# gillette7/Abmarl

Measured on NVIDIA B200. Metric: agent-steps/sec (obs+reward+done) over batched envs, higher is better.
Workload: dtype i8/f64

## Files before the change

### abmarl_b200/csrc/bgw.cu

```cuda
#include <cuda_runtime.h>

#include <algorithm>
#include <cmath>
#include <cstdarg>
#include <cstdio>
#include <cstdlib>
#include <cstring>
#include <vector>

#define BGW_SMALL_KERNELS
#include "bgw_dev.cuh"
#include "bgw_fast.cuh"
#include "bgw_maze.cuh"
#include "bgw_jit.h"

namespace {

thread_local char g_err[2048] = "";

int fail(int code, const char *fmt, ...)
{
    va_list ap;
    va_start(ap, fmt);
    vsnprintf(g_err, sizeof(g_err), fmt, ap);
    va_end(ap);
    return code;
}

#define CUDA_OK(call)                                                                                  \
    do {                                                                                               \
        cudaError_t err__ = (call);                                                                    \
        if (err__ != cudaSuccess) return fail(2, "%s failed: %s", #call, cudaGetErrorString(err__));   \
    } while (0)

struct DeviceGuard {
    int prev = -1;
    explicit DeviceGuard(int dev) { if (cudaGetDevice(&prev) == cudaSuccess && prev != dev) cudaSetDevice(dev); else prev = -1; }
    ~DeviceGuard() { if (prev >= 0) cudaSetDevice(prev); }
};

int align16(int x) { return (x + 15) & ~15; }
int pow2ceil(int x) { int p = 1; while (p < x) p <<= 1; return p; }

}

static const void *observe_fast_fn(int R)
{
    switch (R) {
    case 1: return (const void *)bgw_observe_fast_kernel<1>;
    case 2: return (const void *)bgw_observe_fast_kernel<2>;
    case 3: return (const void *)bgw_observe_fast_kernel<3>;
    case 4: return (const void *)bgw_observe_fast_kernel<4>;
    case 5: return (const void *)bgw_observe_fast_kernel<5>;
    }
    return nullptr;
}

struct BgwEngine {
    int device = 0;
    GeneralStepFn step_fn = nullptr;
    bgwjit::Kernel jit;
    bgwjit::Kernel fast_jit;
    bool fast_jit_on = false;
    const void *fast_fn = nullptr;
    MazeParams maze{};
    bool maze_ok = false, maze_small = false;
    DevSpec ds{}, dsf{};
    FastSpec fs{};
    int threads_fast = 0;
    bool pdl = true;
    bool poisoned = false;
    bool chain_ok = false;
    bool rollout_fused = true;
    bool randomize_action_input = false;
    int16_t *order_buf = nullptr;
    bool use_device_layouts = true;
    uint32_t seq = 0;
    uint32_t *ticket_ring = nullptr;
    std::vector<uint32_t> ticket_next;
    int fast_shape = 0;
    const void *observe_fn = nullptr;
    int observe_grid = 0, observe_smem = 0;
    BgwDims dims{};
    BgwState st{};
    bool bound = false;
    int threads = 0;
    uint64_t launches = 0;
    std::vector<void *> allocs;
};

namespace {

template <typename T>
int upload(BgwEngine *h, const T *src, size_t n, const T **dst)
{
    void *p = nullptr;
    CUDA_OK(cudaMalloc(&p, std::max<size_t>(n, 1) * sizeof(T)));
    h->allocs.push_back(p);
    if (n) CUDA_OK(cudaMemcpy(p, src, n * sizeof(T), cudaMemcpyHostToDevice));
    *dst = (const T *)p;
    return 0;
}

void los_apply_host(uint8_t *mask, int R, int rd, int cd)
{
    const int n = 2 * R + 1;
    if (rd == 0 && cd == 0) return;
    if (cd != 0) {
        double du, dl;
        if (rd == 0) { du = dl = (cd > 0) ? (double)cd - 0.5 : (double)cd + 0.5; }
        else if ((rd > 0) == (cd > 0)) { du = (double)cd - 0.5; dl = (double)cd + 0.5; }
        else { du = (double)cd + 0.5; dl = (double)cd - 0.5; }
        volatile double ku = ((double)rd + 0.5) / du, kl = ((double)rd - 0.5) / dl;
        const int c0 = cd > 0 ? cd : -R, c1 = cd > 0 ? R : cd;
        const int r0 = rd > 0 ? rd : -R, r1 = rd < 0 ? rd : R;
        for (int c = c0; c <= c1; ++c) {
            volatile double up = ku * (double)c, lo = kl * (double)c;
            for (int r = r0; r <= r1; ++r) {
                if (c == cd && r == rd) continue;
                if (lo < (double)r && (double)r < up) mask[(r + R) * n + (c + R)] = 0;
            }
        }
    } else {
        const double d = rd > 0 ? (double)rd - 0.5 : (double)rd + 0.5;
        volatile double kl = ((double)cd - 0.5) / d, kr = ((double)cd + 0.5) / d;
        const int r0 = rd > 0 ? rd : -R, r1 = rd > 0 ? R : rd;
        for (int r = r0; r <= r1; ++r) {
            volatile double le = kl * (double)r, ri = kr * (double)r;
            for (int c = -R; c <= R; ++c) {
                if (c == cd && r == rd) continue;
                if (le < (double)c && (double)c < ri) mask[(r + R) * n + (c + R)] = 0;
            }
        }
    }
}

template <typename Scratch>
__global__ void bgw_layout_kernel(const MazeParams p, const BgwState st, int E, int env_offset, const uint8_t *env_mask, int only_done)
{
    __shared__ Scratch w;
    if (threadIdx.x != 0) return;
    for (int e = blockIdx.x; e < E; e += gridDim.x) {
        if (only_done ? !(st.env_flags[e] & BGW_ENV_ALL_DONE) : (env_mask && !env_mask[e])) continue;
        const int err = maze_layout(p, (uint32_t)(env_offset + e), st.episode[e] + 1u, w, st.layout + (size_t)e * p.A);
        if (err) st.error[e] = (uint32_t)err;
    }
}

int first_role(const BgwSpec *sp, int role)
{
    for (int a = 0; a < sp->n_agents; ++a) if (sp->role[a] == role) return a;
    return -1;
}

}

extern "C" {

const char *bgw_last_error(void) { return g_err; }
int bgw_abi_version(void) { return BGW_ABI_VERSION; }

int bgw_create(const BgwSpec *sp, int device, bgw_handle *out)
{
    if (!sp || !out) return fail(1, "bgw_create: null argument");
    *out = nullptr;
    if (sp->abi_version != BGW_ABI_VERSION) return fail(1, "bgw_create: ABI version %d, library has %d", sp->abi_version, BGW_ABI_VERSION);
    int ndev = 0;
    if (cudaGetDeviceCount(&ndev) != cudaSuccess || ndev == 0)
        return fail(2, "bgw_create: no CUDA device (this engine has no CPU fallback)");
    if (device < 0 || device >= ndev) return fail(1, "bgw_create: device %d out of range (%d devices)", device, ndev);
    const int A = sp->n_agents, H = sp->rows, W = sp->cols, HW = H * W;
    if (A < 1 || A > BGW_MAX_AGENTS) return fail(1, "bgw_create: n_agents %d not in 1..%d", A, BGW_MAX_AGENTS);
    if (H < 1 || W < 1 || HW > BGW_MAX_CELLS) return fail(1, "bgw_create: grid %dx%d not supported (at most %d cells)", H, W, BGW_MAX_CELLS);
    if (sp->n_envs < 1) return fail(1, "bgw_create: n_envs must be positive");

    BgwEngine *h = new BgwEngine();
    h->device = device;
    DeviceGuard guard(device);
    DevSpec &d = h->ds;
    auto bail = [&](int rc) { bgw_destroy(h); return rc; };

    d.H = H; d.W = W; d.HW = HW; d.A = A; d.E = sp->n_envs; d.env_offset = sp->env_offset;
    d.program = sp->program; d.move_actor = sp->move_actor; d.attack_actor = sp->attack_actor;
    d.observer = sp->observer; d.observe_self = sp->observe_self; d.done_mask = sp->done_mask;
    d.manager = sp->manager; d.ravel = sp->ravel_actions; d.no_overlap = sp->no_overlap_at_reset;
    d.stacked = sp->stacked_attacks; d.horizon = sp->horizon; d.auto_reset = sp->auto_reset;
    d.randomize_placement_order = sp->randomize_placement_order;
    d.seed = sp->seed;
    memcpy(d.reward, sp->reward, sizeof(d.reward));

    std::vector<int16_t> learner_of(A, -1), agent_of;
    std::vector<uint16_t> blk, blk_static, var, init_cell(A, BGW_NONE);
    int max_enc = 0, rmax_obs = 0, rmax_att = 0, n_ammo = 0, att_payload = 1;
    for (int a = 0; a < A; ++a) if (sp->encoding[a] > max_enc) max_enc = std::min((int)sp->encoding[a], BGW_MAX_ENCODING);
    if (sp->attack_actor < BGW_ATTACK_NONE || sp->attack_actor > BGW_ATTACK_SELECTIVE) return bail(fail(1, "bgw_create: unknown attack actor %d", sp->attack_actor));
    for (int a = 0; a < A; ++a) {
        const int e = sp->encoding[a];
        if (e < 1 || e > BGW_MAX_ENCODING) return bail(fail(1, "bgw_create: entity %d has encoding %d, must be 1..%d", a, e, BGW_MAX_ENCODING));
        if (sp->target && (sp->target[a] < -1 || sp->target[a] >= A)) return bail(fail(1, "bgw_create: entity %d names target %d, must be -1 or an entity index below %d", a, (int)sp->target[a], A));
        if (sp->klass[a] & BGW_AG_LEARNER) { learner_of[a] = (int16_t)agent_of.size(); agent_of.push_back((int16_t)a); }
        if (sp->klass[a] & BGW_AG_BLOCKING) {
            const bool is_static = !(sp->klass[a] & (BGW_AG_MOVING | BGW_AG_HEALTH)) && sp->init_row[a] >= 0;
            (is_static ? blk_static : blk).push_back((uint16_t)a);
        }
        if (sp->init_row[a] < 0) var.push_back((uint16_t)a);
        else {
            if (sp->init_row[a] >= H || sp->init_col[a] < 0 || sp->init_col[a] >= W)
                return bail(fail(1, "bgw_create: entity %d initial position off the grid", a));
            init_cell[a] = (uint16_t)(sp->init_row[a] * W + sp->init_col[a]);
        }
        if ((sp->klass[a] & BGW_AG_LEARNER) && (sp->klass[a] & BGW_AG_OBSERVING)) {
            int R = sp->view_range[a];
            if (R < 0) return bail(fail(1, "bgw_create: negative view range"));
            rmax_obs = std::max(rmax_obs, R);
        }
        if (sp->klass[a] & BGW_AG_AMMO) {
            ++n_ammo;
            if (!sp->initial_ammo || sp->initial_ammo[a] < 0) return bail(fail(1, "bgw_create: entity %d is an AmmoAgent without a non-negative initial_ammo", a));
        }
        if ((sp->klass[a] & BGW_AG_ATTACKING) && sp->attack_actor != BGW_ATTACK_NONE) {
            const int R = sp->attack_range[a], n = 2 * R + 1, sim = sp->simultaneous_attacks[a];
            rmax_att = std::max(rmax_att, R);
            if (R < 0) return bail(fail(1, "bgw_create: negative attack range"));
            if ((sp->program == BGW_PROG_TEAM_BATTLE || sp->program == BGW_PROG_REACH_TARGET) && sp->attack_actor == BGW_ATTACK_BINARY && sim > 1)
                return bail(fail(1, "bgw_create: TeamBattleSim.step with the BinaryAttackActor is only defined for simultaneous_attacks == 1 (team_battle_example.py:41)"));
            if (sim > BGW_MAX_SIMATT) return bail(fail(1, "bgw_create: simultaneous_attacks %d exceeds %d", sim, BGW_MAX_SIMATT));
            int w = 1, groups = 1;
            if (sp->attack_actor == BGW_ATTACK_ENCODING) { w = max_enc; groups = 0; for (int e = 1; e <= max_enc; ++e) groups += (int)((sp->attack_map[sp->encoding[a]] >> e) & 1); }
            else if (sp->attack_actor == BGW_ATTACK_RESTRICTED) { w = sim; groups = 1; }
            else if (sp->attack_actor == BGW_ATTACK_SELECTIVE) { w = n * n; groups = n * n; }
            if (n * n > 256 && sp->attack_actor >= BGW_ATTACK_RESTRICTED) return bail(fail(1, "bgw_create: attack range %d: a ravelled window cell must fit one byte (range <= 7)", R));
            if (groups * std::max(sim, 1) > BGW_MAX_VICTIMS)
                return bail(fail(1, "bgw_create: entity %d could attack %d agents in one step, the limit is %d", a, groups * sim, BGW_MAX_VICTIMS));
            att_payload = std::max(att_payload, w);
        }
    }
    const int L = (int)agent_of.size();
    if (L < 1) return bail(fail(1, "bgw_create: the simulation has no learning agent"));
    d.n_dyn_blk = (int)blk.size();
    blk.insert(blk.end(), blk_static.begin(), blk_static.end());
    d.L = L; d.max_enc = max_enc; d.n_blk = (int)blk.size(); d.n_var = (int)var.size();
    if (sp->attack_actor != BGW_ATTACK_NONE && d.n_blk > 0 && (2 * rmax_att + 1) * (2 * rmax_att + 1) > 32 * BGW_ATT_MASK_WORDS)
        return bail(fail(1, "bgw_create: attack_range %d with view-blocking entities exceeds the attacker's LOS mask (range <= 7)", rmax_att));
    if (sp->observer == BGW_OBS_STACKED && A > 127) return bail(fail(1, "bgw_create: stacked observer counts are int8 (at most 127 entities)"));
    if (sp->ravel_actions && sp->move_actor != BGW_MOVE_BOX) return bail(fail(1, "bgw_create: ravel_actions needs MoveActor"));

    d.a_nav = first_role(sp, BGW_ROLE_NAVIGATOR); d.a_target = first_role(sp, BGW_ROLE_TARGET);
    d.a_pacman = first_role(sp, BGW_ROLE_PACMAN); d.has_food = first_role(sp, BGW_ROLE_FOOD) >= 0;
    if (sp->program == BGW_PROG_MAZE && (d.a_nav < 0 || d.a_target < 0 || learner_of[d.a_nav] < 0))
        return bail(fail(1, "bgw_create: MazeNavigationSim needs a learning navigator and a target"));
    if (sp->program == BGW_PROG_MULTI_MAZE && d.a_target < 0) return bail(fail(1, "bgw_create: MultiMazeNavigationSim needs a target"));
    for (int k = 0; k < 10; ++k) d.a_script[k] = first_role(sp, BGW_ROLE_SCRIPTED_BADDIE + k);
    if ((sp->program == BGW_PROG_PACMAN || sp->program == BGW_PROG_PACMAN_SIMPLE) && (d.a_pacman < 0 || learner_of[d.a_pacman] < 0 || H <= 9 || W <= 20))
        return bail(fail(1, "bgw_create: PacmanSim needs a learning pacman and the (9,0)<->(9,20) tunnel (pacman.py:87-92)"));
    if (sp->program == BGW_PROG_REACH_TARGET && (d.a_target < 0 || learner_of[d.a_target] < 0))
        return bail(fail(1, "bgw_create: ReachTheTargetSim needs a learning target agent"));
    if (sp->program < BGW_PROG_TEAM_BATTLE || sp->program > BGW_PROG_USER) return bail(fail(1, "bgw_create: unknown program %d", sp->program));
    if (sp->program == BGW_PROG_USER && sp->manager == BGW_MANAGER_DYNAMIC_ORDER)
        return bail(fail(1, "bgw_create: a user step program cannot run under BGW_MANAGER_DYNAMIC_ORDER (its next_agent rule is built in)"));

    BgwDims &dm = h->dims;
    dm.n_envs = d.E; dm.n_agents = A; dm.n_learners = L;
    dm.obs_c = 1;
    if (sp->observer == BGW_OBS_ABSOLUTE) { dm.obs_h = H; dm.obs_w = W; }
    else dm.obs_h = dm.obs_w = 2 * rmax_obs + 1;
    if (sp->observer == BGW_OBS_STACKED) dm.obs_c = max_enc;
    const long long ncell = (long long)dm.obs_h * dm.obs_w * dm.obs_c;
    if (ncell > (1 << 24)) return bail(fail(1, "bgw_create: observation of %lld cells is too large", ncell));
    dm.ammo_offset = -1;
    long long obs_bytes = ncell;
    if (sp->ammo_observer) { dm.ammo_offset = (int)((ncell + 3) / 4 * 4); obs_bytes = dm.ammo_offset + 4; }
    dm.position_offset = -1;
    if (sp->position_observer) { dm.position_offset = (int)((obs_bytes + 3) / 4 * 4); obs_bytes = dm.position_offset + 4; }
    dm.obs_stride = (int)((obs_bytes + 15) / 16 * 16);
    dm.action_stride = (2 + att_payload + 3) / 4 * 4;
    d.act_words = dm.action_stride / 4; d.ammo_offset = dm.ammo_offset; d.n_ammo = n_ammo; d.position_offset = dm.position_offset;
    d.obs_cells = (int)ncell;
    d.obs_h = dm.obs_h; d.obs_w = dm.obs_w; d.obs_c = dm.obs_c; d.obs_stride = dm.obs_stride; d.nchunks = dm.obs_stride / 16;

    d.hw_words = (HW + 31) / 32;
    {
        std::vector<uint16_t> cell(A, BGW_NONE), next(A, BGW_NONE), head(HW, BGW_NONE), tail(HW, BGW_NONE);
        std::vector<uint8_t> flags(A, 0);
        std::vector<uint32_t> avail((size_t)(max_enc + 1) * d.hw_words, 0);
        for (int e = 0; e <= max_enc; ++e)
            for (int i = 0; i < HW; ++i) avail[(size_t)e * d.hw_words + (i >> 5)] |= 1u << (i & 31);
        int err = 0;
        for (int a = 0; a < A; ++a) {
            if (init_cell[a] == BGW_NONE) continue;
            const int c = init_cell[a];
            const uint64_t row = sp->overlap[sp->encoding[a]];
            for (uint16_t o = head[c]; o != BGW_NONE; o = next[o])
                if (!((row >> sp->encoding[o]) & 1)) { err = 1; break; }
            if (tail[c] != BGW_NONE) next[tail[c]] = (uint16_t)a; else head[c] = (uint16_t)a;
            tail[c] = (uint16_t)a; cell[a] = (uint16_t)c; flags[a] = BGW_ST_IN_GRID;
            for (int e = 1; e <= max_enc; ++e)
                if (sp->no_overlap_at_reset || !((row >> e) & 1)) avail[(size_t)e * d.hw_words + (c >> 5)] &= ~(1u << (c & 31));
        }
        d.tpl_error = err;
        int rc;
        if ((rc = upload(h, cell.data(), A, &d.tpl_cell)) || (rc = upload(h, next.data(), A, &d.tpl_next)) ||
            (rc = upload(h, flags.data(), A, &d.tpl_flags)) || (rc = upload(h, avail.data(), avail.size(), &d.tpl_avail)))
            return bail(rc);
    }
    {
        int rc;
        std::vector<unsigned long long> ov(BGW_MAX_ENCODING + 1), am(BGW_MAX_ENCODING + 1);
        for (int i = 0; i <= BGW_MAX_ENCODING; ++i) { ov[i] = sp->overlap[i]; am[i] = sp->attack_map[i]; }
        if ((rc = upload(h, sp->encoding, A, &d.enc)) || (rc = upload(h, sp->klass, A, &d.klass)) ||
            (rc = upload(h, sp->role, A, &d.role)) || (rc = upload(h, sp->init_orient, A, &d.init_orient)) ||
            (rc = upload(h, sp->simultaneous_attacks, A, &d.simatt)) || (rc = upload(h, sp->view_range, A, &d.view_r)) ||
            (rc = upload(h, sp->move_range, A, &d.move_r)) || (rc = upload(h, sp->attack_range, A, &d.attack_r)) ||
            (rc = upload(h, sp->target, A, &d.target)) || (rc = upload(h, learner_of.data(), A, &d.learner_of)) ||
            (rc = upload(h, agent_of.data(), L, &d.agent_of)) || (rc = upload(h, sp->init_health, A, &d.init_health)) ||
            (rc = upload(h, sp->attack_strength, A, &d.strength)) || (rc = upload(h, sp->attack_accuracy, A, &d.accuracy)) ||
            (rc = upload(h, ov.data(), ov.size(), &d.overlap)) || (rc = upload(h, am.data(), am.size(), &d.attack_map)) ||
            (rc = upload(h, blk.data(), blk.size(), &d.blk_agents)) || (rc = upload(h, var.data(), var.size(), &d.var_agents)))
            return bail(rc);
        d.init_ammo = nullptr;
        if (n_ammo && (rc = upload(h, sp->initial_ammo, A, &d.init_ammo))) return bail(rc);
        h->maze_ok = false;
        if (sp->layout_kind == BGW_LAYOUT_MAZE || sp->layout_kind == BGW_LAYOUT_TARGET_BARRIERS_FREE) {
            if (sp->layout_target < 0 || sp->layout_target >= A) return bail(fail(1, "bgw_create: the placement state needs a target agent"));
            MazeParams &m = h->maze;
            m.kind = sp->layout_kind;
            m.rows = H; m.cols = W; m.A = A; m.max_enc = max_enc; m.no_overlap = sp->no_overlap_at_reset; m.target = sp->layout_target;
            m.cluster_barriers = sp->cluster_barriers; m.scatter_free = sp->scatter_free_agents;
            m.seed = sp->seed; m.barrier_encodings = sp->barrier_encodings; m.free_encodings = sp->free_encodings;
            m.enc = d.enc; m.overlap = d.overlap;
            if ((rc = upload(h, sp->init_row, A, &m.init_row)) || (rc = upload(h, sp->init_col, A, &m.init_col))) return bail(rc);
            h->maze_ok = maze_supported(H, W, max_enc, sp->barrier_encodings, sp->free_encodings);
            h->maze_small = maze_fits<MazeScratchSmall>(H, W, max_enc, sp->barrier_encodings, sp->free_encodings);
        } else if (sp->layout_kind != BGW_LAYOUT_POSITION_STATE) return bail(fail(1, "bgw_create: unknown layout_kind %d", sp->layout_kind));
    }

    int T = A <= 128 ? 32 : A <= 1024 ? 64 : 128;
    if (const char *t = getenv("BGW_THREADS")) { const int v = atoi(t); if (v >= 32 && v <= 256 && v % 32 == 0) T = v; }
    h->threads = T;
    d.parallel_actors = ((sp->program == BGW_PROG_TEAM_BATTLE || sp->program == BGW_PROG_REACH_TARGET || sp->program == BGW_PROG_TRAFFIC) && (sp->move_actor == BGW_MOVE_BOX || sp->move_actor == BGW_MOVE_CROSS));
    if (sp->program == BGW_PROG_TRAFFIC)
        for (int a = 0; a < A; ++a) if (sp->target[a] >= 0 && (sp->klass[sp->target[a]] & BGW_AG_MOVING)) d.parallel_actors = 0;
    if (const char *t = getenv("BGW_SERIAL_ACTORS")) if (atoi(t)) d.parallel_actors = 0;
    int slots = std::min(std::max(pow2ceil(HW), 32), 2048);
    if (const char *t = getenv("BGW_SLOTS")) { const int v = atoi(t); if (v >= 32 && v <= 65536 && (v & (v - 1)) == 0) slots = v; }
    d.slot_mask = slots - 1;
    {
        int reff = rmax_obs;
        if (sp->observer == BGW_OBS_ABSOLUTE) reff = std::min(reff, std::max(H, W) - 1);
        const long long nbits = (long long)(2 * reff + 1) * (2 * reff + 1);
        d.mask_words = d.n_blk ? (int)((nbits + 31) / 32) : 0;
        d.mask_batch = 0;
        if (d.n_blk) {
            if ((long long)d.mask_words * 4 > 96 * 1024) return bail(fail(1, "bgw_create: view range %d with view-blocking entities needs a %lld-bit LOS mask, too large for shared memory", reff, nbits));
            d.mask_batch = std::max(1, std::min(L, 32 * 1024 / (d.mask_words * 4)));
        }
        d.static_mask = nullptr;
        bool uniform = true;
        int ru = -1;
        for (int a = 0; a < A; ++a)
            if ((sp->klass[a] & BGW_AG_LEARNER) && (sp->klass[a] & BGW_AG_OBSERVING)) {
                if (ru < 0) ru = sp->view_range[a]; else if (sp->view_range[a] != ru) uniform = false;
            }
        const size_t table_words = (size_t)HW * d.mask_words;
        if (!blk_static.empty() && uniform && ru >= 0 && table_words * 4 <= (64u << 20) && !getenv("BGW_NO_STATIC_MASK")) {
            const int R = reff, n = 2 * R + 1;
            std::vector<uint32_t> table(table_words, 0xFFFFFFFFu);
            std::vector<uint8_t> one((size_t)n * n);
            for (int c = 0; c < HW; ++c) {
                uint32_t *row = table.data() + (size_t)c * d.mask_words;
                const int r0 = c / W, c0 = c % W;
                for (uint16_t b : blk_static) {
                    const int rd = sp->init_row[b] - r0, cd = sp->init_col[b] - c0;
                    if (rd < -R || rd > R || cd < -R || cd > R) continue;
                    memset(one.data(), 1, one.size());
                    los_apply_host(one.data(), R, rd, cd);
                    for (int i = 0; i < n * n; ++i) if (!one[i]) row[i >> 5] &= ~(1u << (i & 31));
                }
            }
            int rc = upload(h, table.data(), table.size(), &d.static_mask);
            if (rc) return bail(rc);
        }
    }
    int off = 0;
    auto take = [&](int bytes) { const int o = off; off += align16(bytes); return o; };
    d.o_head = take(HW * 2 + 2);
    d.o_slot = take(slots * 4);
    d.o_cell = take(A * 2); d.o_next = take(A * 2);
    d.o_flags = take(A); d.o_enc = take(A); d.o_klass = take(A); d.o_tmp = take(A);
    d.o_racc = take(A * 8);
    d.o_act = take(L * dm.action_stride);
    d.o_ragent = take(L * 2); d.o_plist = take(L * 2); d.o_pstate = take(L);
    d.o_avail = take((max_enc + 1) * d.hw_words * 4);
    d.o_mask = take(d.mask_batch * d.mask_words * 4);
    d.o_ctr = take(CTR_COUNT * 4);
    d.o_csum = take(HW);
    {
        FastSpec &f = h->fs;
        const int P = std::max(rmax_obs, rmax_att);
        bool fast = sp->program == BGW_PROG_TEAM_BATTLE && sp->manager == BGW_MANAGER_ALL_STEP &&
                    (sp->move_actor == BGW_MOVE_BOX || sp->move_actor == BGW_MOVE_CROSS) && d.n_blk == 0 &&
                    sp->observer == BGW_OBS_POSITION_CENTERED && sp->attack_actor == BGW_ATTACK_BINARY && n_ammo == 0 &&
                    !sp->ammo_observer && !sp->position_observer &&
                    (2 * rmax_att + 1) * (2 * rmax_att + 1) <= 32;
        if (const char *t = getenv("BGW_GENERIC_KERNEL")) if (atoi(t)) fast = false;
        int TF = A <= 32 ? 32 : A <= 64 ? 64 : 96;
        if (A == FastStaticC5::A && H == FastStaticC5::H && W == FastStaticC5::W) TF = FastStaticC5::T;
        if (const char *t = getenv("BGW_THREADS")) { const int v = atoi(t); if (v >= 32 && v <= 1024 && v % 32 == 0) TF = std::min(v, 128); }
        if (fast) {
            f.P = P;
            f.PL = P;
            f.PW = (W + 2 * P + 3) / 4 * 4;
            f.PH = H + 2 * P;
            f.magic_w = (uint32_t)(((1ull << 32) + (uint64_t)W - 1) / (uint64_t)W);
            int fslots = std::min(std::max(pow2ceil(HW), 32), 256);
            if (const char *t = getenv("BGW_SLOTS")) { const int v = atoi(t); if (v >= 32 && v <= 65536 && (v & (v - 1)) == 0) fslots = v; }
            h->dsf = d;
            h->dsf.slot_mask = fslots - 1;
            const long long cbytes = (long long)f.PH * f.PW + 32;
            const FastLayout ly = fast_layout(A, L, HW, f.PH, f.PW, fslots, TF, max_enc, d.hw_words, L == A);
            fast_apply_layout(f, ly);
            const int fo = ly.smem_bytes;
            f.async_ok = (A % 16 == 0) ? 1 : (A % 8 == 0) ? 2 : 0;
            f.simd_ok = (A % 4 == 0);
            f.uniform_view = -1;
            bool first = true, uniform = true;
            for (int a = 0; a < A; ++a)
                if ((sp->klass[a] & BGW_AG_LEARNER) && (sp->klass[a] & BGW_AG_OBSERVING)) {
                    if (first) { f.uniform_view = sp->view_range[a]; first = false; }
                    else if (sp->view_range[a] != f.uniform_view) uniform = false;
                }
            if (!uniform) f.uniform_view = -1;
            f.uniform_att = -1;
            {
                bool firsta = true, unia = true;
                for (int a = 0; a < A; ++a)
                    if (sp->klass[a] & BGW_AG_ATTACKING) {
                        if (firsta) { f.uniform_att = sp->attack_range[a]; firsta = false; }
                        else if (sp->attack_range[a] != f.uniform_att) unia = false;
                    }
                if (!unia) f.uniform_att = -1;
            }
            f.identity_learners = (L == A);
            {
                unsigned long long present = 0;
                for (int a = 0; a < A; ++a) present |= 1ull << sp->encoding[a];
                f.can_mix = 0; f.acc_lt1 = 0;
                for (int e = 1; e <= max_enc; ++e)
                    if (((present >> e) & 1ull) && (sp->overlap[e] & present & ~(1ull << e))) f.can_mix = 1;
                for (int a = 0; a < A; ++a)
                    if ((sp->klass[a] & BGW_AG_ATTACKING) && sp->attack_accuracy[a] < 1.0) f.acc_lt1 = 1;
            }
            f.epoch0 = 0xFFFFEu;
            if (const char *t = getenv("BGW_EPOCH0")) { const long v = atol(t); if (v >= 1 && v <= 0xFFFFE) f.epoch0 = (uint32_t)v; }
            if (cbytes > 96 * 1024 || fo > 227 * 1024) fast = false;
        }
        f.enabled = fast;
        h->threads_fast = TF;
        if (fast) {
            h->fast_shape = fast_shape_matches<FastStaticC5>(h->dsf, f, TF) ? 1 : fast_shape_matches<FastStaticC2>(h->dsf, f, TF) ? 2 : 0;
            if (const char *t = getenv("BGW_DYNAMIC_SHAPES")) if (atoi(t)) h->fast_shape = 0;
            h->fast_fn = bgw_fast_step_fn(h->fast_shape, f.head_elem);
        }
    }
    d.smem_bytes = off;
    if (off > 227 * 1024) return bail(fail(1, "bgw_create: one environment needs %d bytes of shared memory (limit 232448): grid or entity count too large", off));
    cudaError_t ce;
    h->step_fn = d.program == BGW_PROG_USER ? nullptr : bgw_general_step_fn(d.program, d.attack_actor);
    if (const char *t = getenv("BGW_ALL_IN_ONE_KERNEL")) if (atoi(t) && h->step_fn) h->step_fn = bgw_general_step_fn(-1, -1);
    if ((h->step_fn && (ce = cudaFuncSetAttribute(h->step_fn, cudaFuncAttributeMaxDynamicSharedMemorySize, off)) != cudaSuccess) ||
        (h->fs.enabled && (ce = cudaFuncSetAttribute(h->fast_fn, cudaFuncAttributeMaxDynamicSharedMemorySize, h->fs.smem_bytes)) != cudaSuccess) ||
        (ce = cudaFuncSetAttribute(bgw_reset_kernel, cudaFuncAttributeMaxDynamicSharedMemorySize, off)) != cudaSuccess ||
        (ce = cudaFuncSetAttribute(bgw_observe_kernel, cudaFuncAttributeMaxDynamicSharedMemorySize, off)) != cudaSuccess)
        return bail(fail(2, "bgw_create: cudaFuncSetAttribute: %s", cudaGetErrorString(ce)));
    if (h->fs.enabled && !h->fs.can_mix && sp->observe_self && h->fs.uniform_view >= 1 && h->fs.uniform_view <= 5 && !getenv("BGW_GENERIC_OBSERVE")) {
        const ObserveLayout lay = observe_layout(d.A, d.L, h->fs.PH, h->fs.PW);
        int per_sm = 0, sms = 0;
        h->observe_fn = observe_fast_fn(h->fs.uniform_view);
        h->observe_smem = lay.bytes;
        if ((ce = cudaFuncSetAttribute(h->observe_fn, cudaFuncAttributeMaxDynamicSharedMemorySize, lay.bytes)) != cudaSuccess ||
            (ce = cudaOccupancyMaxActiveBlocksPerMultiprocessor(&per_sm, h->observe_fn, 128, (size_t)lay.bytes)) != cudaSuccess ||
            (ce = cudaDeviceGetAttribute(&sms, cudaDevAttrMultiProcessorCount, device)) != cudaSuccess)
            return bail(fail(2, "bgw_create: observe kernel set-up: %s", cudaGetErrorString(ce)));
        h->observe_grid = std::max(1, std::min(d.E, per_sm * sms));
        if (const char *t = getenv("BGW_OBSERVE_GRID")) { const int v = atoi(t); if (v >= 1) h->observe_grid = std::min(d.E, v); }
    }
    if (getenv("BGW_VERBOSE")) {
        if (h->observe_fn) fprintf(stderr, "[bgw] observe kernel: gather-only, view %d\n", h->fs.uniform_view);
        else fprintf(stderr, "[bgw] observe kernel: general\n");
    }
    if (h->fs.enabled) {
        int per_sm = 0, sms = 0;
        ce = cudaOccupancyMaxActiveBlocksPerMultiprocessor(&per_sm, h->fast_fn, h->threads_fast, (size_t)h->fs.smem_bytes);
        if (ce != cudaSuccess ||
            (ce = cudaDeviceGetAttribute(&sms, cudaDevAttrMultiProcessorCount, device)) != cudaSuccess)
            return bail(fail(2, "bgw_create: occupancy query: %s", cudaGetErrorString(ce)));
        h->fs.grid_ctas = std::max(1, std::min(d.E, per_sm * sms));
        if (getenv("BGW_PROF_FILE")) {
            void *pp = nullptr;
            if (cudaMalloc(&pp, (size_t)h->fs.grid_ctas * 8 * 16 * sizeof(long long)) == cudaSuccess) { h->allocs.push_back(pp); cudaMemset(pp, 0, (size_t)h->fs.grid_ctas * 8 * 16 * sizeof(long long)); h->fs.prof = (long long *)pp; }
        }
        if (getenv("BGW_VERBOSE")) fprintf(stderr, "[bgw] fast kernel: shape %s, T=%d smem=%d B/CTA, %d CTAs/SM x %d SMs, grid=%d, slots=%d\n", h->fast_shape == 1 ? "C5 (compile-time)" : h->fast_shape == 2 ? "C2 (compile-time)" : "run-time", h->threads_fast, h->fs.smem_bytes, per_sm, sms, h->fs.grid_ctas, h->dsf.slot_mask + 1);
        if (const char *t = getenv("BGW_PDL")) h->pdl = atoi(t) != 0;
        if (const char *t = getenv("BGW_GRID")) { const int v = atoi(t); if (v >= 1) h->fs.grid_ctas = std::min(d.E, v); }
        {
            void *pp = nullptr;
            const size_t nb = ((size_t)d.E + BGW_TICKET_RING) * sizeof(uint32_t);
            if ((ce = cudaMalloc(&pp, nb)) != cudaSuccess || (ce = cudaMemset(pp, 0, nb)) != cudaSuccess)
                return bail(fail(2, "bgw_create: env stamps: %s", cudaGetErrorString(ce)));
            h->allocs.push_back(pp);
            h->ticket_ring = (uint32_t *)pp;
            h->fs.env_seq = (uint32_t *)pp + BGW_TICKET_RING;
        }
        h->chain_ok = h->pdl && !(h->maze_ok && sp->auto_reset);
        if (const char *t = getenv("BGW_CHAIN")) if (!atoi(t)) h->chain_ok = false;
        if (const char *t = getenv("BGW_ROLLOUT_FUSED")) h->rollout_fused = atoi(t) != 0;
        h->fs.wait_limit_ns = 10ull * 1000ull * 1000ull * 1000ull;
        if (const char *t = getenv("BGW_WAIT_LIMIT_MS")) { const long long v = atoll(t); if (v > 0) h->fs.wait_limit_ns = (unsigned long long)v * 1000000ull; }
    }
    if (sp->randomize_action_input) {
        if (sp->manager != BGW_MANAGER_ALL_STEP) return bail(fail(1, "bgw_create: randomize_action_input is an AllStepManager option (all_step_manager.py:24-35)"));
        void *pp = nullptr;
        if ((ce = cudaMalloc(&pp, (size_t)d.E * std::max(L, 1) * sizeof(int16_t))) != cudaSuccess)
            return bail(fail(2, "bgw_create: order buffer: %s", cudaGetErrorString(ce)));
        h->allocs.push_back(pp);
        h->order_buf = (int16_t *)pp;
        h->randomize_action_input = true;
    }
    dm.device_layouts = h->maze_ok ? 1 : 0;
    dm.threads_per_env = h->fs.enabled ? h->threads_fast : T; dm.envs_per_cta = 1; dm.smem_bytes = h->fs.enabled ? h->fs.smem_bytes : off;
    *out = h;
    return 0;
}

int bgw_destroy(bgw_handle h)
{
    if (!h) return 0;
    DeviceGuard guard(h->device);
    if (h->jit.module) bgwjit::driver().ModuleUnload(h->jit.module);
    if (h->fast_jit.module) bgwjit::driver().ModuleUnload(h->fast_jit.module);
    for (void *p : h->allocs) cudaFree(p);
    delete h;
    return 0;
}

int bgw_specialize(bgw_handle h, const char *cache_dir)
{
    if (!h) return fail(1, "bgw_specialize: null handle");
    if (h->jit.function || h->fast_jit.function) return 0;
    if (h->ds.program == BGW_PROG_USER) return 0;
    if (h->fs.enabled && (h->fast_shape != 0 || (h->bound && h->st.layout) || h->fs.prof)) return 0;
    DeviceGuard guard(h->device);
    CUDA_OK(cudaFree(nullptr));
    if (!cache_dir) cache_dir = getenv("BGW_JIT_CACHE");
    std::string msg;
    if (!h->fs.enabled) {
        if (const char *e = bgwjit::build(h->ds, h->ds.init_ammo != nullptr, h->threads, cache_dir, h->jit, msg))
            return fail(2, "bgw_specialize: %s", e);
        return 0;
    }
    const int by_smem = (228 * 1024) / (h->fs.smem_bytes + 1024), by_regs = 65536 / (h->threads_fast * 72);
    const int lb_n = std::max(1, std::min(32, std::min(by_smem, by_regs)));
    if (const char *e = bgwjit::build_fast(h->dsf, h->fs, h->threads_fast, lb_n, cache_dir, h->fast_jit, msg))
        return fail(2, "bgw_specialize: %s", e);
    int per_sm = 0, sms = 0;
    const int rc = bgwjit::driver().OccupancyMaxActiveBlocks(&per_sm, h->fast_jit.function, h->threads_fast, (size_t)h->fs.smem_bytes);
    if (rc || per_sm < 1) { bgwjit::driver().ModuleUnload(h->fast_jit.module); h->fast_jit = bgwjit::Kernel(); return fail(2, "bgw_specialize: occupancy query of the compiled kernel failed (%d)", rc); }
    CUDA_OK(cudaDeviceGetAttribute(&sms, cudaDevAttrMultiProcessorCount, h->device));
    h->fs.grid_ctas = std::max(1, std::min(h->ds.E, per_sm * sms));
    if (const char *t = getenv("BGW_GRID")) { const int v = atoi(t); if (v >= 1) h->fs.grid_ctas = std::min(h->ds.E, v); }
    h->fast_jit_on = true;
    if (getenv("BGW_VERBOSE")) fprintf(stderr, "[bgw] fast kernel compiled for this spec's shape: %d CTAs/SM, grid=%d\n", per_sm, h->fs.grid_ctas);
    return 0;
}

int bgw_set_program(bgw_handle h, const char *source, const char *cache_dir)
{
    if (!h || !source) return fail(1, "bgw_set_program: null argument");
    if (h->ds.program != BGW_PROG_USER) return fail(1, "bgw_set_program: the handle's spec runs built-in program %d, not BGW_PROG_USER", h->ds.program);
    if (h->jit.function) return fail(1, "bgw_set_program: the handle has a step program already");
    DeviceGuard guard(h->device);
    CUDA_OK(cudaFree(nullptr));
    if (!cache_dir) cache_dir = getenv("BGW_JIT_CACHE");
    std::string msg;
    if (const char *e = bgwjit::build(h->ds, h->ds.init_ammo != nullptr, h->threads, cache_dir, h->jit, msg, source))
        return fail(2, "bgw_set_program: %s", e);
    return 0;
}

int bgw_dims(bgw_handle h, BgwDims *out)
{
    if (!h || !out) return fail(1, "bgw_dims: null argument");
    *out = h->dims;
    return 0;
}

int bgw_bind_state(bgw_handle h, const BgwState *state)
{
    if (!h || !state) return fail(1, "bgw_bind_state: null argument");
    if (!state->cell || !state->next || !state->flags || !state->health || !state->reward_acc || !state->episode ||
        !state->step || !state->env_flags || !state->turn || !state->error || !state->stats)
        return fail(1, "bgw_bind_state: every array except `layout` and `ammo` is required");
    if (h->ds.n_ammo && !state->ammo) return fail(1, "bgw_bind_state: the simulation has AmmoAgents: `ammo` is required");
    h->st = *state;
    h->bound = true;
    if (state->layout && h->fs.enabled && (h->fast_shape != 0 || h->fast_jit_on)) {
        h->fast_jit_on = false;
        DeviceGuard guard(h->device);
        h->fast_shape = 0;
        h->fast_fn = bgw_fast_step_fn(0, h->fs.head_elem);
        CUDA_OK(cudaFuncSetAttribute(h->fast_fn, cudaFuncAttributeMaxDynamicSharedMemorySize, h->fs.smem_bytes));
        int per_sm = 0, sms = 0;
        CUDA_OK(cudaOccupancyMaxActiveBlocksPerMultiprocessor(&per_sm, h->fast_fn, h->threads_fast, (size_t)h->fs.smem_bytes));
        CUDA_OK(cudaDeviceGetAttribute(&sms, cudaDevAttrMultiProcessorCount, h->device));
        h->fs.grid_ctas = std::max(1, std::min(h->ds.E, per_sm * sms));
    }
    return 0;
}

int bgw_reset(bgw_handle h, const uint8_t *env_mask, int8_t *obs, void *stream)
{
    if (!h) return fail(1, "bgw_reset: null handle");
    if (!h->bound) return fail(1, "bgw_reset: call bgw_bind_state first");
    DeviceGuard guard(h->device);
    bgw_reset_kernel<<<h->ds.E, h->threads, h->ds.smem_bytes, (cudaStream_t)stream>>>(h->ds, h->st, env_mask, obs);
    CUDA_OK(cudaGetLastError());
    h->launches += 1;
    return 0;
}

int bgw_observe(bgw_handle h, const uint8_t *env_mask, int8_t *obs, void *stream)
{
    if (!h) return fail(1, "bgw_observe: null handle");
    if (!h->bound) return fail(1, "bgw_observe: call bgw_bind_state first");
    if (!obs) return fail(1, "bgw_observe: obs is null");
    DeviceGuard guard(h->device);
    if (h->observe_fn) {
        void *args[] = {(void *)&h->dsf, (void *)&h->fs, (void *)&h->st, (void *)&env_mask, (void *)&obs};
        CUDA_OK(cudaLaunchKernel(h->observe_fn, dim3(h->observe_grid), dim3(128), args, (size_t)h->observe_smem, (cudaStream_t)stream));
    } else {
        bgw_observe_kernel<<<h->ds.E, h->threads, h->ds.smem_bytes, (cudaStream_t)stream>>>(h->ds, h->st, env_mask, obs);
        CUDA_OK(cudaGetLastError());
    }
    h->launches += 1;
    return 0;
}

static void dump_prof(bgw_handle h, void *stream)
{
    const size_t n = (size_t)h->fs.grid_ctas * 8 * 16;
    std::vector<long long> host(n);
    cudaStreamSynchronize((cudaStream_t)stream);
    cudaMemcpy(host.data(), h->fs.prof, n * sizeof(long long), cudaMemcpyDeviceToHost);
    if (FILE *fp = fopen(getenv("BGW_PROF_FILE"), "wb")) { fwrite(host.data(), sizeof(long long), n, fp); fclose(fp); }
}

static int step_impl(bgw_handle h, const int8_t *actions, int8_t *sampled, const int16_t *order, int8_t *obs, float *reward,
                     uint8_t *done, uint8_t *all_done, void *stream, bool chained = false, int n_steps = 1)
{
    if (h->ds.program == BGW_PROG_USER && !h->jit.function)
        return fail(1, "bgw_step: the handle runs a user step program and none is installed yet (bgw_set_program)");
    DeviceGuard guard(h->device);
    if (h->randomize_action_input && !order) {
        if (n_steps != 1) return fail(1, "bgw_step: randomize_action_input needs one launch per step");
        const int L = h->ds.L, P = pow2ceil(std::max(L, 2));
        bgw_order_kernel<<<h->ds.E, std::min(1024, std::max(32, P / 2)), (size_t)P * sizeof(unsigned long long), (cudaStream_t)stream>>>(h->ds, h->st, P, h->order_buf);
        CUDA_OK(cudaGetLastError());
        h->launches += 1;
        order = h->order_buf;
        chained = false;
    }
    if (h->fs.enabled) {
        if (h->poisoned) return fail(2, "bgw_step: an earlier step launch failed; the handle cannot be used any more");
        {
            const cudaError_t pe = cudaPeekAtLastError();
            if (pe != cudaSuccess) { h->poisoned = true; return fail(2, "bgw_step: an earlier launch failed on the device (%s); the handle cannot be used any more", cudaGetErrorString(pe)); }
        }
        cudaStreamCaptureStatus capture = cudaStreamCaptureStatusNone;
        CUDA_OK(cudaStreamIsCapturing((cudaStream_t)stream, &capture));
        if (capture != cudaStreamCaptureStatusNone && n_steps != 1) return fail(1, "bgw_step: a captured launch is one manager step");
        h->fs.seq = h->seq + 1u;
        h->seq += (uint32_t)n_steps;
        h->fs.n_tickets = (uint32_t)n_steps * (uint32_t)h->ds.E;
        if (capture != cudaStreamCaptureStatusNone) {
            h->fs.chain = 0; h->fs.ticket = nullptr; h->fs.ticket_base = 0;
        } else {
            h->fs.chain = (chained && h->chain_ok) ? 1 : 0;
            if (h->ticket_next.empty()) h->ticket_next.assign(BGW_TICKET_RING, 0u);
            const uint32_t slot = h->fs.seq % BGW_TICKET_RING;
            h->fs.ticket = h->ticket_ring + slot;
            h->fs.ticket_base = h->ticket_next[slot];
            h->ticket_next[slot] += h->fs.n_tickets + (uint32_t)h->fs.grid_ctas;
        }
        h->poisoned = true;
        cudaLaunchAttribute pdl_attr[1];
        pdl_attr[0].id = cudaLaunchAttributeProgrammaticStreamSerialization;
        pdl_attr[0].val.programmaticStreamSerializationAllowed = h->pdl ? 1 : 0;
        cudaLaunchConfig_t cfg = {};
        cfg.gridDim = dim3((unsigned)h->fs.grid_ctas); cfg.blockDim = dim3((unsigned)h->threads_fast);
        cfg.dynamicSmemBytes = (size_t)h->fs.smem_bytes; cfg.stream = (cudaStream_t)stream;
        cfg.attrs = pdl_attr; cfg.numAttrs = 1;
        const uint32_t *act_arg = (const uint32_t *)actions;
        uint32_t *smp_arg = (uint32_t *)sampled;
        void *args[] = {&h->dsf, &h->fs, &h->st, &act_arg, &smp_arg, &order, &obs, &reward, &done, &all_done};
        if (h->fast_jit_on) {
            CUlaunchAttribute ja[1];
            memset(ja, 0, sizeof(ja));
            ja[0].id = CU_LAUNCH_ATTRIBUTE_PROGRAMMATIC_STREAM_SERIALIZATION;
            ja[0].value.programmaticStreamSerializationAllowed = h->pdl ? 1 : 0;
            CUlaunchConfig jc;
            memset(&jc, 0, sizeof(jc));
            jc.gridDimX = (unsigned)h->fs.grid_ctas; jc.gridDimY = jc.gridDimZ = 1;
            jc.blockDimX = (unsigned)h->threads_fast; jc.blockDimY = jc.blockDimZ = 1;
            jc.sharedMemBytes = (unsigned)h->fs.smem_bytes; jc.hStream = (CUstream)stream; jc.attrs = ja; jc.numAttrs = 1;
            const int rc = bgwjit::driver().LaunchKernelEx(&jc, h->fast_jit.function, args, nullptr);
            if (rc) { const char *es = nullptr; bgwjit::driver().GetErrorString(rc, &es); return fail(2, "bgw_step: cuLaunchKernelEx of the specialised kernel: %s", es ? es : "?"); }
        } else
            CUDA_OK(cudaLaunchKernelExC(&cfg, h->fast_fn, args));
        h->poisoned = false;
    } else {
        if (sampled) {
            const size_t n = (size_t)h->ds.E * h->ds.L;
            bgw_sample_actions_kernel<<<(unsigned)((n + 255) / 256), 256, 0, (cudaStream_t)stream>>>(h->ds, h->st, (uint32_t *)sampled);
            CUDA_OK(cudaGetLastError());
            h->launches += 1;
            actions = sampled;
        }
        if (h->jit.function) {
            const uint32_t *act_arg = (const uint32_t *)actions;
            void *args[] = {&h->ds, &h->st, &act_arg, &order, &obs, &reward, &done, &all_done};
            const int rc = bgwjit::driver().LaunchKernel(h->jit.function, (unsigned)h->ds.E, 1, 1, (unsigned)h->threads, 1, 1,
                                                         (unsigned)h->ds.smem_bytes, stream, args, nullptr);
            if (rc) { const char *es = nullptr; bgwjit::driver().GetErrorString(rc, &es); return fail(2, "bgw_step: cuLaunchKernel of the specialised kernel: %s", es ? es : "?"); }
        } else
            h->step_fn<<<h->ds.E, h->threads, h->ds.smem_bytes, (cudaStream_t)stream>>>(
                h->ds, h->st, (const uint32_t *)actions, order, obs, reward, done, all_done);
    }
    CUDA_OK(cudaGetLastError());
    h->launches += 1;
    if (h->fs.enabled && h->fs.prof && !getenv("BGW_PROF_LAZY")) dump_prof(h, stream);
    return 0;
}

int bgw_step(bgw_handle h, const int8_t *actions, const int16_t *order, int8_t *obs, float *reward, uint8_t *done,
             uint8_t *all_done, void *stream)
{
    if (!h) return fail(1, "bgw_step: null handle");
    if (!h->bound) return fail(1, "bgw_step: call bgw_bind_state first");
    if (!actions || !reward || !done || !all_done) return fail(1, "bgw_step: actions, reward, done and all_done are required");
    return step_impl(h, actions, nullptr, order, obs, reward, done, all_done, stream);
}

int bgw_step_sampled(bgw_handle h, int8_t *actions_out, const int16_t *order, int8_t *obs, float *reward, uint8_t *done,
                     uint8_t *all_done, void *stream)
{
    if (!h) return fail(1, "bgw_step_sampled: null handle");
    if (!h->bound) return fail(1, "bgw_step_sampled: call bgw_bind_state first");
    if (!actions_out || !reward || !done || !all_done) return fail(1, "bgw_step_sampled: actions_out, reward, done and all_done are required");
    return step_impl(h, nullptr, actions_out, order, obs, reward, done, all_done, stream);
}

int bgw_rollout_sampled(bgw_handle h, int n_steps, int8_t *actions_out, const int16_t *order, int8_t *obs, float *reward,
                        uint8_t *done, uint8_t *all_done, void *stream)
{
    if (!h) return fail(1, "bgw_rollout_sampled: null handle");
    if (!h->bound) return fail(1, "bgw_rollout_sampled: call bgw_bind_state first");
    if (n_steps < 0) return fail(1, "bgw_rollout_sampled: n_steps < 0");
    if (!actions_out || !reward || !done || !all_done) return fail(1, "bgw_rollout_sampled: actions_out, reward, done and all_done are required");
    const bool layouts_between = h->maze_ok && h->st.layout && h->ds.auto_reset && h->use_device_layouts;
    cudaStreamCaptureStatus capture = cudaStreamCaptureStatusNone;
    if (h->fs.enabled) {
        DeviceGuard guard(h->device);
        CUDA_OK(cudaStreamIsCapturing((cudaStream_t)stream, &capture));
        if (capture == cudaStreamCaptureStatusNone) {
            const cudaError_t qe = cudaStreamQuery((cudaStream_t)stream);
            if (qe != cudaSuccess && qe != cudaErrorNotReady) { h->poisoned = true; return fail(2, "bgw_rollout_sampled: the stream reports %s; the handle cannot be used any more", cudaGetErrorString(qe)); }
        }
    }
    if (h->fs.enabled && h->rollout_fused && !layouts_between && !(h->randomize_action_input && !order) && capture == cudaStreamCaptureStatusNone) {
        const int kmax = std::max(1, (int)(0x7FFFFFFFu / (uint32_t)h->ds.E) - 1);
        for (int i = 0; i < n_steps; i += kmax) {
            const int rc = step_impl(h, nullptr, actions_out, order, obs, reward, done, all_done, stream, i > 0, std::min(kmax, n_steps - i));
            if (rc) return rc;
        }
    } else {
        for (int i = 0; i < n_steps; ++i) {
            const int rc = step_impl(h, nullptr, actions_out, order, obs, reward, done, all_done, stream, i > 0 && !layouts_between);
            if (rc) return rc;
            if (layouts_between) {
                const int rl = bgw_generate_layouts(h, nullptr, 1, stream);
                if (rl) return rl;
            }
        }
    }
    if (h->fs.enabled && h->fs.prof && getenv("BGW_PROF_LAZY")) dump_prof(h, stream);
    return 0;
}

int bgw_sample_actions(bgw_handle h, int8_t *actions, void *stream)
{
    if (!h || !actions) return fail(1, "bgw_sample_actions: null argument");
    if (!h->bound) return fail(1, "bgw_sample_actions: call bgw_bind_state first");
    DeviceGuard guard(h->device);
    const size_t n = (size_t)h->ds.E * h->ds.L;
    bgw_sample_actions_kernel<<<(unsigned)((n + 255) / 256), 256, 0, (cudaStream_t)stream>>>(h->ds, h->st, (uint32_t *)actions);
    CUDA_OK(cudaGetLastError());
    h->launches += 1;
    return 0;
}

int bgw_gather_valid(bgw_handle h, const int8_t *obs, const float *reward, const uint8_t *done, const uint8_t *all_done,
                     int32_t *count, int32_t *index, int8_t *obs_c, float *reward_c, uint8_t *done_c, void *stream)
{
    if (!h || !obs || !reward || !done || !all_done || !count || !index || !obs_c || !reward_c || !done_c)
        return fail(1, "bgw_gather_valid: null argument");
    DeviceGuard guard(h->device);
    CUDA_OK(cudaMemsetAsync(count, 0, sizeof(int32_t), (cudaStream_t)stream));
    const int L = h->ds.L;
    bgw_gather_kernel<<<h->ds.E, 128, 16 + align16(L * 2), (cudaStream_t)stream>>>(
        L, h->ds.obs_stride, obs, reward, done, all_done, count, index, obs_c, reward_c, done_c);
    CUDA_OK(cudaGetLastError());
    h->launches += 1;
    return 0;
}

int bgw_generate_layouts(bgw_handle h, const uint8_t *env_mask, int only_done, void *stream)
{
    if (!h) return fail(1, "bgw_generate_layouts: null handle");
    if (!h->maze_ok) return fail(1, "bgw_generate_layouts: this simulation has no device-side layout generator (BgwDims.device_layouts == 0)");
    if (!h->bound || !h->st.layout) return fail(1, "bgw_generate_layouts: bind a state with a `layout` array first");
    DeviceGuard guard(h->device);
    int sms = 148;
    cudaDeviceGetAttribute(&sms, cudaDevAttrMultiProcessorCount, h->device);
    if (h->maze_small)
        bgw_layout_kernel<MazeScratchSmall><<<std::min(h->ds.E, sms * 32), 32, 0, (cudaStream_t)stream>>>(h->maze, h->st, h->ds.E, h->ds.env_offset, env_mask, only_done);
    else
        bgw_layout_kernel<MazeScratch><<<std::min(h->ds.E, sms * 15), 32, 0, (cudaStream_t)stream>>>(h->maze, h->st, h->ds.E, h->ds.env_offset, env_mask, only_done);
    CUDA_OK(cudaGetLastError());
    h->launches += 1;
    return 0;
}

int bgw_use_device_layouts(bgw_handle h, int on)
{
    if (!h) return fail(1, "bgw_use_device_layouts: null handle");
    if (on && !h->maze_ok) return fail(1, "bgw_use_device_layouts: this simulation has no device-side layout generator");
    h->use_device_layouts = on != 0;
    return 0;
}

int bgw_maze_layout_host(const BgwSpec *sp, uint32_t global_env, uint32_t episode, uint16_t *layout)
{
    if (!sp || !layout) return fail(1, "bgw_maze_layout_host: null argument");
    if (sp->layout_kind != BGW_LAYOUT_MAZE && sp->layout_kind != BGW_LAYOUT_TARGET_BARRIERS_FREE)
        return fail(1, "bgw_maze_layout_host: the spec has no MazePlacementState / TargetBarriersFreePlacementState");
    int max_enc = 0;
    for (int a = 0; a < sp->n_agents; ++a) max_enc = std::max(max_enc, (int)sp->encoding[a]);
    if (!maze_supported(sp->rows, sp->cols, max_enc, sp->barrier_encodings, sp->free_encodings))
        return fail(1, "bgw_maze_layout_host: grid or encoding count above the generator's limits");
    std::vector<unsigned long long> ov(BGW_MAX_ENCODING + 1);
    for (int i = 0; i <= BGW_MAX_ENCODING; ++i) ov[i] = sp->overlap[i];
    MazeParams m{};
    m.kind = sp->layout_kind;
    m.rows = sp->rows; m.cols = sp->cols; m.A = sp->n_agents; m.max_enc = max_enc; m.no_overlap = sp->no_overlap_at_reset;
    m.target = sp->layout_target; m.cluster_barriers = sp->cluster_barriers; m.scatter_free = sp->scatter_free_agents;
    m.seed = sp->seed; m.barrier_encodings = sp->barrier_encodings; m.free_encodings = sp->free_encodings;
    m.enc = sp->encoding; m.init_row = sp->init_row; m.init_col = sp->init_col; m.overlap = ov.data();
    std::vector<MazeScratch> w(1);
    const int err = maze_layout(m, global_env, episode, w[0], layout);
    return err ? fail(10 + err, "bgw_maze_layout_host: no cell available for an entity (state.py:598-603)") : 0;
}

int bgw_rng_draw(uint64_t seed, uint32_t env, uint32_t episode, uint32_t step, uint32_t site, uint32_t slot, uint32_t k,
                 uint32_t out[4])
{
    bgw_draw4(seed, env, episode, step, site, slot, k, out);
    return 0;
}

int bgw_los_mask(int range, int r_diff, int c_diff, uint8_t *out)
{
    if (range < 0 || !out) return fail(1, "bgw_los_mask: bad argument");
    const int n = 2 * range + 1;
    memset(out, 1, (size_t)n * n);
    if (r_diff < -range || r_diff > range || c_diff < -range || c_diff > range) return 0;
    los_apply_host(out, range, r_diff, c_diff);
    return 0;
}

uint64_t bgw_launch_count(bgw_handle h) { return h ? h->launches : 0; }

}
```

### abmarl_b200/csrc/bgw_fast.cuh

```cuda
#pragma once
#include "bgw_dev.cuh"

#define BGW_MIXED (-128)
#ifdef BGW_JITTER
__device__ __forceinline__ void bgw_jitter(unsigned site)
{
    unsigned x = (unsigned)clock64() * 2654435761u + threadIdx.x * 40503u + site * 2246822519u;
    x ^= x >> 15; x *= 2246822519u; x ^= x >> 13;
    if (x & 3u) __nanosleep(x & 0x7FFu);
}
#define BGW_JITTER_POINT(site) bgw_jitter(site)
#else
#define BGW_JITTER_POINT(site) do { } while (0)
#endif
#ifdef BGW_PROFILE
#define BGW_PROF_MARK(k) do { if (f.prof && tid == 0 && it_no < 8) f.prof[((size_t)blockIdx.x * 8 + it_no) * 16 + (k)] = clock64(); } while (0)
#else
#define BGW_PROF_MARK(k) do { } while (0)
#endif

struct FastSpec {
    int enabled;
    int P, PL, PW, PH;
    uint32_t magic_w;
    int uniform_view;
    int uniform_att;
    int identity_learners;
    int can_mix;
    int acc_lt1;
    int grid_ctas;
    int async_ok;
    int simd_ok;
    uint32_t epoch0;
    int b_cell, b_next, b_flags, buf_bytes;
    int o_enc, o_klass, o_tmp, o_act, o_head, o_cenc, o_rel, o_ragent, o_plist, o_ctr, o_wsum, o_buf, o_scratch;
    int s_rflag, s_slot, s_rkmask, s_eff, s_pstate, s_killrank, s_touch, scratch_bytes, smem_bytes;
    int touch_words;
    int r_racc, r_avail;
    int head_elem;
    long long *prof;
    uint32_t *env_seq;
    uint32_t *ticket;
    uint32_t ticket_base;
    uint32_t seq;
    uint32_t n_tickets;
    unsigned long long wait_limit_ns;
    int chain;
};

struct FastLayout {
    int b_cell, b_next, b_flags, buf_bytes;
    int o_enc, o_klass, o_tmp, o_act, o_head, o_cenc, o_rel, o_ragent, o_plist, o_ctr, o_wsum, o_buf, o_scratch;
    int s_rflag, s_slot, s_rkmask, s_eff, s_pstate, s_killrank, s_touch, touch_words, scratch_bytes, smem_bytes;
    int r_racc, r_avail, head_elem;
};

__host__ __device__ constexpr int fl_align16(int x) { return (x + 15) & ~15; }
__host__ __device__ constexpr int fl_touch_words(int HW)
{
    int w = 4;
    while (w * 32 < HW && w < 128) w <<= 1;
    return w;
}

__host__ __device__ constexpr FastLayout fast_layout(int A, int L, int HW, int PH, int PW, int slots, int T, int max_enc,
                                                     int hw_words, int identity)
{
    FastLayout y{};
    int fo = 0;
    y.o_enc = fo; fo += fl_align16(A);
    y.o_klass = fo; fo += fl_align16(A);
    y.o_tmp = fo; fo += fl_align16(A);
    y.o_rel = fo; fo += fl_align16(A * 2);
    y.o_ragent = fo; fo += fl_align16(L * 2);
    y.o_plist = identity ? y.o_ragent : fo;
    if (!identity) fo += fl_align16(L * 2);
    y.o_act = fo; fo += fl_align16(L * 4);
    y.o_ctr = fo; fo += fl_align16(CTR_COUNT * 4);
    y.o_wsum = fo; fo += fl_align16(32 * 4);
    int bo = 0;
    y.b_cell = bo; bo += fl_align16(A * 2);
    y.b_next = bo; bo += fl_align16(A * 2);
    y.b_flags = bo; bo += fl_align16(A);
    y.buf_bytes = bo;
    y.o_buf = fo; fo += 2 * bo;
    int so = 0;
    y.s_rkmask = so; so += fl_align16(L * 4);
    y.s_eff = so; so += fl_align16(L * 2);
    y.s_pstate = so; so += fl_align16(L);
    y.s_killrank = so; so += fl_align16(A * 2);
    y.s_slot = so; so += fl_align16(slots * 4);
    y.touch_words = fl_touch_words(HW);
    y.s_touch = so; so += 2 * y.touch_words * 4;
    y.s_rflag = so; so += fl_align16(A);
    const int actor_bytes = so;
    const int cenc_bytes = fl_align16(PH * PW + 32);
    y.head_elem = A <= 256 ? 1 : 2;
    const int head_bytes = fl_align16(HW * y.head_elem + 2);
    y.r_racc = fl_align16(HW * 2 + 2);
    y.r_avail = y.r_racc + fl_align16(A * 8);
    const int reset_bytes = y.r_avail + fl_align16((max_enc + 1) * hw_words * 4);
    int sb = actor_bytes;
    if (reset_bytes - cenc_bytes - head_bytes > sb) sb = reset_bytes - cenc_bytes - head_bytes;
    y.scratch_bytes = sb;
    y.o_cenc = fo; fo += cenc_bytes;
    y.o_head = fo; fo += head_bytes;
    y.o_scratch = fo; fo += sb;
    y.smem_bytes = fo;
    return y;
}

__host__ __device__ inline void fast_apply_layout(FastSpec &f, const FastLayout &y)
{
    f.b_cell = y.b_cell; f.b_next = y.b_next; f.b_flags = y.b_flags; f.buf_bytes = y.buf_bytes;
    f.o_enc = y.o_enc; f.o_klass = y.o_klass; f.o_tmp = y.o_tmp; f.o_act = y.o_act; f.o_head = y.o_head;
    f.o_cenc = y.o_cenc; f.o_rel = y.o_rel; f.o_ragent = y.o_ragent; f.o_plist = y.o_plist; f.o_ctr = y.o_ctr;
    f.o_wsum = y.o_wsum; f.o_buf = y.o_buf; f.o_scratch = y.o_scratch;
    f.s_rflag = y.s_rflag; f.s_slot = y.s_slot; f.s_rkmask = y.s_rkmask; f.s_eff = y.s_eff; f.s_pstate = y.s_pstate;
    f.s_killrank = y.s_killrank; f.s_touch = y.s_touch; f.touch_words = y.touch_words; f.scratch_bytes = y.scratch_bytes; f.smem_bytes = y.smem_bytes;
    f.r_racc = y.r_racc; f.r_avail = y.r_avail; f.head_elem = y.head_elem;
}

enum { RF_ATTACK_FAIL = 1, RF_KILL = 2, RF_DIED = 4, RF_MOVE_FAIL = 8 };

struct FastEnv {
    void *head;
    uint8_t *rflag;
    int8_t *cenc;
    uint16_t *killrank, *eff, *rel;
    uint32_t *rkmask, *act;
    uint32_t *touch;
    int *wsum;
};

__device__ __forceinline__ void cell_rc(const DevSpec &s, const FastSpec &f, int cell, int &r, int &c)
{
    r = (int)__umulhi((uint32_t)cell, f.magic_w);
    c = cell - r * s.W;
}

__device__ __forceinline__ int pad_index(const DevSpec &s, const FastSpec &f, int cell)
{
    int r, c;
    cell_rc(s, f, cell, r, c);
    return (r + f.P) * f.PW + (c + f.PL);
}

template <typename HT>
__device__ __forceinline__ unsigned fl_first(const FastEnv &fe, int cell, int pidx)
{
    return fe.cenc[pidx] != 0 ? (unsigned)((const HT *)fe.head)[cell] : BGW_NONE16;
}

__device__ __forceinline__ int8_t fl_summary(const Env &ev, unsigned first, bool can_mix)
{
    if (first == BGW_NONE16) return 0;
    const int8_t e = ev.enc[first];
    if (can_mix)
        for (unsigned o = ev.next[first]; o != BGW_NONE16; o = ev.next[o]) if (ev.enc[o] != e) return (int8_t)BGW_MIXED;
    return e;
}

template <typename HT>
__device__ __forceinline__ unsigned fl_unlink(Env &ev, FastEnv &fe, int a)
{
    const int cell = ev.cell[a];
    unsigned first = ((const HT *)fe.head)[cell];
    if (first == (unsigned)a) {
        first = ev.next[a];
        if (first != BGW_NONE16) ((HT *)fe.head)[cell] = (HT)first;
    } else {
        unsigned p = first;
        while (ev.next[p] != (unsigned)a) p = ev.next[p];
        ev.next[p] = ev.next[a];
    }
    ev.next[a] = BGW_NONE16;
    ev.flags[a] &= ~BGW_ST_IN_GRID;
    return first;
}

template <typename HT>
__device__ __forceinline__ void fl_append(Env &ev, FastEnv &fe, int a, int cell, bool occupied)
{
    ev.next[a] = BGW_NONE16;
    if (!occupied) ((HT *)fe.head)[cell] = (HT)a;
    else {
        unsigned p = ((const HT *)fe.head)[cell];
        for (unsigned q = ev.next[p]; q != BGW_NONE16; q = ev.next[p]) p = q;
        ev.next[p] = (uint16_t)a;
    }
    ev.cell[a] = (uint16_t)cell;
    ev.flags[a] |= BGW_ST_IN_GRID;
}

__device__ __forceinline__ void cp_async16(void *smem_dst, const void *gmem_src)
{
    const unsigned d = (unsigned)__cvta_generic_to_shared(smem_dst);
    asm volatile("cp.async.cg.shared.global [%0], [%1], 16;\n" ::"r"(d), "l"(gmem_src) : "memory");
}
__device__ __forceinline__ void cp_async8(void *smem_dst, const void *gmem_src)
{
    const unsigned d = (unsigned)__cvta_generic_to_shared(smem_dst);
    asm volatile("cp.async.ca.shared.global [%0], [%1], 8;\n" ::"r"(d), "l"(gmem_src) : "memory");
}
__device__ __forceinline__ void cp_async_commit() { asm volatile("cp.async.commit_group;\n" ::: "memory"); }
template <int N> __device__ __forceinline__ void cp_async_wait() { asm volatile("cp.async.wait_group %0;\n" ::"n"(N) : "memory"); }

#define BGW_TICKET_RING 2048
__device__ __forceinline__ uint32_t ld_acquire_u32(const uint32_t *p)
{
    uint32_t v;
    asm volatile("ld.acquire.gpu.global.u32 %0, [%1];" : "=r"(v) : "l"(p) : "memory");
    return v;
}
__device__ __forceinline__ void st_release_u32(uint32_t *p, uint32_t v)
{
    asm volatile("st.release.gpu.global.u32 [%0], %1;" ::"l"(p), "r"(v) : "memory");
}
__device__ __forceinline__ bool env_stamped(const FastSpec &f, int e, uint32_t need)
{
    BGW_JITTER_POINT(6);
    return (int32_t)(ld_acquire_u32(f.env_seq + e) - need) >= 0;
}
__device__ __forceinline__ unsigned long long global_timer_ns()
{
    unsigned long long t;
    asm volatile("mov.u64 %0, %%globaltimer;" : "=l"(t));
    return t;
}
__device__ __forceinline__ void env_wait_stamp(const FastSpec &f, int e, uint32_t need)
{
    unsigned spins = 0;
    unsigned long long t0 = 0;
    while (!env_stamped(f, e, need)) {
        __nanosleep(64);
        if ((++spins & 1023u) == 0) {
            const unsigned long long now = global_timer_ns();
            if (t0 == 0) t0 = now;
            else if (now - t0 > f.wait_limit_ns) __trap();
        }
    }
}
#define BGW_TSLOT 12

__device__ __forceinline__ void fast_issue_env(const DevSpec &s, const FastSpec &f, const BgwState &st, const uint32_t *actions,
                                               int e, unsigned char *buf, int tid, int T)
{
    if (actions)
        for (int i = tid; i < (s.L * 4 + 127) / 128; i += T)
            asm volatile("prefetch.global.L2 [%0];" ::"l"((const char *)(actions + (size_t)e * s.L) + (size_t)i * 128));
    const size_t off = (size_t)e * s.A;
    if (f.async_ok == 2) {
        const unsigned char *g;
        g = (const unsigned char *)(st.cell + off);
        for (int i = tid; i < s.A / 4; i += T) cp_async8(buf + f.b_cell + i * 8, g + i * 8);
        g = (const unsigned char *)(st.next + off);
        for (int i = tid; i < s.A / 4; i += T) cp_async8(buf + f.b_next + i * 8, g + i * 8);
        g = (const unsigned char *)(st.flags + off);
        for (int i = tid; i < s.A / 8; i += T) cp_async8(buf + f.b_flags + i * 8, g + i * 8);
    } else if (f.async_ok) {
        const unsigned char *g;
        g = (const unsigned char *)(st.cell + off);
        for (int i = tid; i < s.A / 8; i += T) cp_async16(buf + f.b_cell + i * 16, g + i * 16);
        g = (const unsigned char *)(st.next + off);
        for (int i = tid; i < s.A / 8; i += T) cp_async16(buf + f.b_next + i * 16, g + i * 16);
        g = (const unsigned char *)(st.flags + off);
        for (int i = tid; i < s.A / 16; i += T) cp_async16(buf + f.b_flags + i * 16, g + i * 16);
    } else {
        uint16_t *c = (uint16_t *)(buf + f.b_cell), *n = (uint16_t *)(buf + f.b_next);
        uint8_t *fl = buf + f.b_flags;
        for (int a = tid; a < s.A; a += T) { c[a] = st.cell[off + a]; n[a] = st.next[off + a]; fl[a] = st.flags[off + a]; }
    }
}

template <typename HT>
__device__ void fast_exec_attack(const DevSpec &s, const FastSpec &f, Env &ev, FastEnv &fe, int rank, int a, uint32_t mask)
{
    if (!(ev.flags[a] & BGW_ST_ACTIVE)) return;
    const int R = f.uniform_att >= 0 ? f.uniform_att : __ldg(&s.attack_r[a]), n = 2 * R + 1;
    const int own = ev.cell[a];
    const unsigned long long row = __ldg(&s.attack_map[ev.enc[a]]);
    const double acc = f.acc_lt1 ? __ldg(&s.accuracy[a]) : 1.0;
    int ncand = 0, v = -1, vcell = 0;
    for (uint32_t m = mask; m; m &= m - 1) {
        const int b = __ffs(m) - 1, wr = b / n, wc = b - wr * n;
        const int cc = own + (wr - R) * s.W + (wc - R);
        for (unsigned o = fl_first<HT>(fe, cc, pad_index(s, f, cc)); o != BGW_NONE16; o = ev.next[o])
            if (basic_criteria(s, ev, a, (int)o, row, acc) && ncand++ == 0) { v = (int)o; vcell = cc; }
    }
    if (ncand == 0) { fe.rflag[a] |= RF_ATTACK_FAIL; return; }
    if (ncand > 1) {
        int j = (int)bgw_index(dev_draw(s, ev, BGW_SITE_SUBSET, (uint32_t)a, 0), (uint32_t)ncand);
        v = -1;
        for (uint32_t m = mask; m && v < 0; m &= m - 1) {
            const int b = __ffs(m) - 1, wr = b / n, wc = b - wr * n;
            vcell = own + (wr - R) * s.W + (wc - R);
            for (unsigned o = fl_first<HT>(fe, vcell, pad_index(s, f, vcell)); o != BGW_NONE16; o = ev.next[o])
                if (basic_criteria(s, ev, a, (int)o, row, acc) && j-- == 0) { v = (int)o; break; }
        }
    }
    {
        const double hit = __ldg(&s.strength[a]);
        set_health(ev, v, hit >= 1.0 ? 0.0 : __ldcg(&ev.health[v]) - hit);
    }
    if (!(ev.flags[v] & BGW_ST_ACTIVE)) {
        fe.cenc[pad_index(s, f, vcell)] = fl_summary(ev, fl_unlink<HT>(ev, fe, v), f.can_mix);
        fe.killrank[v] = (uint16_t)rank;
        atomicAdd(&ev.ctr[CTR_KILLS], 1);
        fe.rflag[v] |= RF_DIED;
        fe.rflag[a] |= RF_KILL;
    }
}

#define BGW_TAG_SHIFT 12

struct SlotTables {
    uint32_t *t0, *t1;
    uint32_t mask;
    __device__ __forceinline__ uint32_t *tab(int p) const { return p ? t1 : t0; }
};

__device__ __forceinline__ SlotTables slot_tables(const DevSpec &s, const Env &ev)
{
    SlotTables t;
    const uint32_t half = (uint32_t)(s.slot_mask + 1) >> 1;
    t.t0 = ev.slot; t.t1 = ev.slot + half; t.mask = half - 1u;
    return t;
}

__device__ __forceinline__ void attack_reserve(const DevSpec &s, uint32_t *tab, uint32_t smask, int own, int R, uint32_t mask, uint32_t v)
{
    const int n = 2 * R + 1;
    BGW_JITTER_POINT(1);
    atomicMin(&tab[own & smask], v);
    for (uint32_t m = mask; m; m &= m - 1) {
        const int b = __ffs(m) - 1, wr = b / n, wc = b - wr * n;
        atomicMin(&tab[(own + (wr - R) * s.W + (wc - R)) & smask], v);
    }
}

__device__ __forceinline__ bool attack_holds(const DevSpec &s, const uint32_t *tab, uint32_t smask, int own, int R, uint32_t mask, uint32_t v)
{
    const int n = 2 * R + 1;
    BGW_JITTER_POINT(2);
    bool win = tab[own & smask] == v;
    for (uint32_t m = mask; m; m &= m - 1) {
        const int b = __ffs(m) - 1, wr = b / n, wc = b - wr * n;
        win &= tab[(own + (wr - R) * s.W + (wc - R)) & smask] == v;
    }
    return win;
}

#ifdef BGW_ROUNDS_FIRST
#define BGW_ROUNDS_WARP(T) 0
#else
#define BGW_ROUNDS_WARP(T) (((T) >> 5) - 1)
#endif
#ifndef BGW_BOOK_TID
#define BGW_BOOK_TID 0
#endif
#ifdef BGW_COMPACT_LAST
#define BGW_COMPACT_WARP(T) (((T) >> 5) - 1)
#else
#define BGW_COMPACT_WARP(T) 0
#endif

template <bool WARP, typename HT>
__device__ uint32_t fast_attack_rounds(const DevSpec &s, const FastSpec &f, Env &ev, FastEnv &fe, int n_eff, uint32_t epoch, int tid, int T)
{
    const int stride = WARP ? 32 : T;
    const SlotTables st = slot_tables(s, ev);
    int pending = 1, p = 0;
    while (pending) {
        const uint32_t tag = epoch << BGW_TAG_SHIFT, next_tag = (epoch - 1u) << BGW_TAG_SHIFT;
        int lost = 0;
        for (int x = tid; x < n_eff; x += stride) {
            const int i = fe.eff[x];
            if (ev.pstate[i] != 1) continue;
            const int a = ev.ragent[i], R = f.uniform_att >= 0 ? f.uniform_att : __ldg(&s.attack_r[a]), own = ev.cell[a];
            const uint32_t mask = fe.rkmask[i];
            if (!attack_holds(s, st.tab(p), st.mask, own, R, mask, tag | (uint32_t)i)) {
                lost = 1;
                attack_reserve(s, st.tab(p ^ 1), st.mask, own, R, mask, next_tag | (uint32_t)i);
                continue;
            }
            BGW_JITTER_POINT(9);
            fast_exec_attack<HT>(s, f, ev, fe, i, a, mask);
            ev.pstate[i] = 0;
        }
        if (WARP) { pending = __any_sync(0xFFFFFFFFu, lost); __syncwarp(); } else pending = __syncthreads_or(lost);
        p ^= 1; --epoch;
    }
    return epoch;
}

template <typename HT>
__device__ __forceinline__ void fast_exec_move(const DevSpec &s, const FastSpec &f, Env &ev, FastEnv &fe, int a, int from, int to)
{
    const int pto = pad_index(s, f, to);
    const int8_t summary = fe.cenc[pto], me = ev.enc[a];
    const unsigned fl = ev.flags[a], hd = ((const HT *)fe.head)[from], nx = ev.next[a];
    if ((summary == 0) & ((fl & BGW_ST_IN_GRID) != 0) & (hd == (unsigned)a) & (nx == BGW_NONE16)) {
        fe.cenc[pad_index(s, f, from)] = 0;
        fe.cenc[pto] = me;
        ((HT *)fe.head)[to] = (HT)a;
        ev.cell[a] = (uint16_t)to;
        return;
    }
    bool ok = true;
    if (summary != 0) {
        const unsigned long long row = __ldg(&s.overlap[me]);
        if (!f.can_mix || summary != (int8_t)BGW_MIXED) ok = (row >> summary) & 1ull;
        else
            for (unsigned o = ((const HT *)fe.head)[to]; o != BGW_NONE16; o = ev.next[o])
                if (!((row >> ev.enc[o]) & 1ull)) { ok = false; break; }
    }
    if (!ok) { fe.rflag[a] |= RF_MOVE_FAIL; return; }
    if (fl & BGW_ST_IN_GRID) fe.cenc[pad_index(s, f, from)] = fl_summary(ev, fl_unlink<HT>(ev, fe, a), f.can_mix);
    fl_append<HT>(ev, fe, a, to, summary != 0);
    const int8_t ns = (!f.can_mix || summary == 0 || summary == me) ? me : (int8_t)BGW_MIXED;
    fe.cenc[pto] = ns;
    if (f.can_mix && ns == (int8_t)BGW_MIXED) ev.ctr[CTR_MIXED] = 1;
}

#define BGW_NO_MOVE 0xFFFFFFFFu
__device__ __forceinline__ void touch_mark(const FastSpec &f, FastEnv &fe, int cell)
{
    BGW_JITTER_POINT(3);
    const uint32_t bit = 1u << (cell & 31);
    uint32_t *w = fe.touch + ((cell >> 5) & (f.touch_words - 1));
    if (atomicOr(w, bit) & bit) atomicOr(w + f.touch_words, bit);
}

template <bool WARP, typename HT>
__device__ uint32_t fast_move_rounds(const DevSpec &s, const FastSpec &f, Env &ev, FastEnv &fe, int n_cur, uint32_t epoch, int tid, int T)
{
    const int stride = WARP ? 32 : T;
    const SlotTables st = slot_tables(s, ev);
    uint32_t *cur = st.t0, *nxt = st.t1;
    int which = 0, base0 = 0, base1 = 0;
    int pending = 1;
    while (pending) {
        const uint32_t tag = epoch << BGW_TAG_SHIFT, next_tag = (epoch - 1u) << BGW_TAG_SHIFT;
        const uint16_t *walk = which ? fe.killrank : fe.eff;
        uint16_t *losers = which ? fe.eff : fe.killrank;
        int *lctr = &ev.ctr[CTR_PA + (which ^ 1)];
        const int lbase = which ? base0 : base1;
        int lost = 0;
        for (int x = tid; x < n_cur; x += stride) {
            const int i = walk[x];
            const uint32_t ft = fe.rkmask[i];
            const int from = (int)(ft >> 16), to = (int)(ft & 0xFFFFu);
            const uint32_t mine = tag | (uint32_t)i, sf = (uint32_t)from & st.mask, sto = (uint32_t)to & st.mask;
            BGW_JITTER_POINT(4);
            const uint32_t hf = cur[sf], ht = cur[sto];
            if ((hf != mine) | (ht != mine)) {
                lost = 1;
                atomicMin(&nxt[sf], next_tag | (uint32_t)i);
                atomicMin(&nxt[sto], next_tag | (uint32_t)i);
                losers[atomicAdd(lctr, 1) - lbase] = (uint16_t)i;
                continue;
            }
            fast_exec_move<HT>(s, f, ev, fe, ev.ragent[i], from, to);
        }
        if (WARP) { pending = __any_sync(0xFFFFFFFFu, lost); __syncwarp(); }
        else pending = __syncthreads_or(lost);
        if (which) base1 += n_cur; else base0 += n_cur;
        n_cur = *(volatile int *)lctr - lbase;
        which ^= 1;
        { uint32_t *t = cur; cur = nxt; nxt = t; }
        --epoch;
    }
    return epoch;
}

template <typename HT>
__device__ uint32_t fast_move_phase(const DevSpec &s, const FastSpec &f, Env &ev, FastEnv &fe, int n_act, uint32_t epoch, int tid, int T)
{
    const SlotTables st = slot_tables(s, ev);
    const uint32_t *twice = fe.touch + f.touch_words;
    const uint32_t tw = (uint32_t)f.touch_words - 1u, tag = epoch << BGW_TAG_SHIFT;
    for (int i = tid; i < n_act; i += T) {
        const uint32_t ft = fe.rkmask[i];
        if (ft == BGW_NO_MOVE) continue;
        const int from = (int)(ft >> 16), to = (int)(ft & 0xFFFFu);
        BGW_JITTER_POINT(5);
        const uint32_t c = (twice[((uint32_t)from >> 5) & tw] >> (from & 31)) | (twice[((uint32_t)to >> 5) & tw] >> (to & 31));
        if (c & 1u) {
            fe.eff[atomicAdd(&ev.ctr[CTR_PA], 1)] = (uint16_t)i;
            atomicMin(&st.t0[(uint32_t)from & st.mask], tag | (uint32_t)i);
            atomicMin(&st.t0[(uint32_t)to & st.mask], tag | (uint32_t)i);
        } else {
            fast_exec_move<HT>(s, f, ev, fe, ev.ragent[i], from, to);
        }
    }
    __syncthreads();
    {
        uint4 *t4 = reinterpret_cast<uint4 *>(fe.touch);
        for (int w = tid; w < f.touch_words / 2; w += T) t4[w] = make_uint4(0, 0, 0, 0);
    }
    const int n_con = ev.ctr[CTR_PA];
    if (n_con > 0) {
        if ((tid >> 5) == BGW_ROUNDS_WARP(T)) {
            const uint32_t e2 = fast_move_rounds<true, HT>(s, f, ev, fe, n_con, epoch, tid & 31, T);
            if ((tid & 31) == 0) ev.ctr[CTR_EPOCH] = (int)e2;
        }
        __syncthreads();
        return (uint32_t)ev.ctr[CTR_EPOCH];
    }
    return epoch;
}

static __device__ void fast_init_dense(const DevSpec &s, const FastSpec &f, Env &ev, FastEnv &fe, int tid, int T)
{
    const uint4 ones = make_uint4(0xFFFFFFFFu, 0xFFFFFFFFu, 0xFFFFFFFFu, 0xFFFFFFFFu);
    for (int a = tid; a < s.A; a += T) ev.tmp[a] = 0;
    {
        uint4 *s4 = (uint4 *)ev.slot;
        for (int i = tid; i < (s.slot_mask + 1) / 4; i += T) s4[i] = ones;
        uint4 *t4 = (uint4 *)fe.touch;
        for (int i = tid; i < f.touch_words / 2; i += T) t4[i] = make_uint4(0, 0, 0, 0);
    }
    uint32_t *c32 = (uint32_t *)fe.cenc;
    const int wpr = f.PW >> 2, lane = tid & 31, warp = tid >> 5, nwarp = T >> 5;
    for (int cw = lane; cw < wpr; cw += 32) {
        uint32_t inner = 0xFFFFFFFFu;
#pragma unroll
        for (int bb = 0; bb < 4; ++bb) {
            const int cc = cw * 4 + bb;
            if (cc >= f.PL && cc < f.PL + s.W) inner &= ~(0xFFu << (8 * bb));
        }
        for (int rr = warp; rr < f.PH; rr += nwarp)
            c32[rr * wpr + cw] = (rr >= f.P && rr < f.P + s.H) ? inner : 0xFFFFFFFFu;
    }
    if (tid < 8) c32[f.PH * wpr + tid] = 0xFFFFFFFFu;
    __syncthreads();
}

template <typename HT>
__device__ void fast_obs_chunk_slow(const DevSpec &s, const FastSpec &f, const Env &ev, const FastEnv &fe, int a, int ch,
                                    uint32_t w[4])
{
    w[0] = w[1] = w[2] = w[3] = 0;
    if (!(ev.klass[a] & BGW_AG_OBSERVING)) return;
    const int R = __ldg(&s.view_r[a]), n = 2 * R + 1, valid = n * n, k0 = ch * 16;
    int r0, c0;
    cell_rc(s, f, ev.cell[a], r0, c0);
    const int8_t *win = fe.cenc + (r0 + f.P - R) * f.PW + (c0 + f.PL - R);
    int wr = k0 / n, wc = k0 - wr * n;
    for (int t = 0; t < 16 && k0 + t < valid; ++t) {
        int v = win[wr * f.PW + wc];
        const bool centre = (wr == R && wc == R);
        if (v == BGW_MIXED || (centre && !s.observe_self && v > 0)) {
            const int cell = (r0 - R + wr) * s.W + (c0 - R + wc), skip = s.observe_self ? -1 : a;
            const unsigned first = ((const HT *)fe.head)[cell];
            int cnt = 0;
            for (unsigned o = first; o != BGW_NONE16; o = ev.next[o]) cnt += ((int)o != skip);
            v = 0;
            if (cnt > 0) {
                int k = (cnt == 1) ? 0 : (int)bgw_index(dev_draw(s, ev, BGW_SITE_OBS, (uint32_t)a, (uint32_t)cell), (uint32_t)cnt);
                for (unsigned o = first; o != BGW_NONE16; o = ev.next[o]) {
                    if ((int)o == skip) continue;
                    if (k-- == 0) { v = ev.enc[o]; break; }
                }
            }
        }
        w[t >> 2] |= (uint32_t)(uint8_t)(int8_t)v << ((t & 3) * 8);
        if (++wc == n) { wc = 0; ++wr; }
    }
}

__device__ __forceinline__ void st_global_256(void *p, const uint32_t *v)
{
#ifdef BGW_NO_ST256
    reinterpret_cast<uint4 *>(p)[0] = make_uint4(v[0], v[1], v[2], v[3]);
    reinterpret_cast<uint4 *>(p)[1] = make_uint4(v[4], v[5], v[6], v[7]);
    return;
#endif
    asm volatile("st.global.v8.b32 [%0], {%1, %2, %3, %4, %5, %6, %7, %8};" ::"l"(p), "r"(v[0]), "r"(v[1]), "r"(v[2]), "r"(v[3]),
                 "r"(v[4]), "r"(v[5]), "r"(v[6]), "r"(v[7])
                 : "memory");
}

template <int R> struct ObsCoop { static constexpr bool on = false; static constexpr int LPA = 1, a = 0, b = 0, NR = 0; };
template <> struct ObsCoop<5> { static constexpr bool on = true; static constexpr int LPA = 4, a = 3, b = -1, NR = 4; };
template <> struct ObsCoop<3> { static constexpr bool on = true; static constexpr int LPA = 2, a = 4, b = 0, NR = 5; };

template <int R>
__host__ __device__ constexpr int obs_coop_lo(int r)
{
    typedef ObsCoop<R> C;
    const int n = 2 * R + 1;
    int lo = n;
    for (int q = 0; q < C::LPA; ++q) {
        const int st = 32 * q - n * (C::a * q + C::b) - n * r;
        const int l = st < 0 ? 0 : st;
        if (l < lo && st + 32 > 0 && st < n) lo = l;
    }
    return lo;
}
template <int R>
__host__ __device__ constexpr int obs_coop_hi(int r)
{
    typedef ObsCoop<R> C;
    const int n = 2 * R + 1;
    int hi = 0;
    for (int q = 0; q < C::LPA; ++q) {
        const int st = 32 * q - n * (C::a * q + C::b) - n * r;
        const int h = st + 32 > n ? n : st + 32;
        if (h > hi && st + 32 > 0 && st < n) hi = h;
    }
    return hi;
}

template <int R>
__device__ void fast_obs_rows_coop(const DevSpec &s, const FastSpec &f, const Env &ev, const FastEnv &fe, int n_act, int8_t *obs_env,
                                   int tid, int T)
{
    typedef ObsCoop<R> C;
    constexpr int n = 2 * R + 1, LPA = C::LPA, NR = C::NR;
    constexpr int RW = (n + 3) / 4;
    constexpr int LW = (n + 6) / 4;
    constexpr int ST0 = -n * C::b, SLOPE = 32 - n * C::a;
    constexpr int ST_MIN = SLOPE >= 0 ? ST0 : ST0 + SLOPE * (LPA - 1);
    constexpr int W0 = ST_MIN / 4;
    constexpr int SW = W0 + 9;
    static_assert(ST_MIN >= 0 && (SLOPE >= 0 ? ST0 + SLOPE * (LPA - 1) : ST0) - 4 * W0 <= 4, "lane-dependent shift must stay within 0..4 bytes");
    static_assert((NR * n + 3) / 4 <= SW, "stream longer than the extraction window");
    const int q = tid & (LPA - 1);
    const int dyn = (ST0 + SLOPE * q - 4 * W0) * 8;
    const int pw4 = f.PW >> 2;
    const bool wide = ((s.obs_stride & 31) == 0) && ((reinterpret_cast<uintptr_t>(obs_env) & 31) == 0);
    for (int li = tid / LPA; li < n_act; li += T / LPA) {
        const int a = ev.ragent[li];
        const bool observing = ev.klass[a] & BGW_AG_OBSERVING;
        const int i0 = C::a * q + C::b;
        const int o = pad_index(s, f, ev.cell[a]) - R * f.PW - R;
        const uint32_t *wp = reinterpret_cast<const uint32_t *>(fe.cenc + (o & ~3)) + i0 * pw4;
        const int sh = (o & 3) * 8;
        uint32_t S[SW + 1];
#pragma unroll
        for (int j = 0; j <= SW; ++j) S[j] = 0;
        if (observing) {
#pragma unroll
            for (int r = 0; r < NR; ++r) {
                const int lo = obs_coop_lo<R>(r), hi = obs_coop_hi<R>(r);
                if (hi <= lo) continue;
                const bool ok = (unsigned)(i0 + r) < (unsigned)n;
                const uint32_t *rp = wp + r * pw4;
                uint32_t x[LW + 1], y[RW];
#pragma unroll
                for (int j = 0; j <= LW; ++j) {
                    const bool ny = j < RW && !(4 * j + 4 <= lo || 4 * j >= hi);
                    const bool nyp = j > 0 && j - 1 < RW && !(4 * (j - 1) + 4 <= lo || 4 * (j - 1) >= hi);
                    if (j < LW && (ny || nyp)) x[j] = (ok && (j < LW - 1 || sh + 8 * n > 32 * (LW - 1))) ? rp[j] : 0u;
                    else x[j] = 0;
                }
#pragma unroll
                for (int j = 0; j < RW; ++j)
                    y[j] = (4 * j + 4 <= lo || 4 * j >= hi) ? 0u : __funnelshift_r(x[j], x[j + 1], sh);
                constexpr int vb = n - 4 * (RW - 1);
                if (vb < 4) y[RW - 1] &= (1u << (8 * (vb & 3))) - 1u;
                const int d = n * r, qw = d >> 2, s8 = (d & 3) * 8;
#pragma unroll
                for (int j = 0; j < RW; ++j) {
                    if (4 * j + 4 <= lo || 4 * j >= hi) continue;
                    if (qw + j <= SW) S[qw + j] |= y[j] << s8;
                    if (s8 != 0 && qw + j + 1 <= SW) S[qw + j + 1] |= y[j] >> (32 - s8);
                }
            }
        }
        uint32_t out[8];
#pragma unroll
        for (int j = 0; j < 8; ++j) out[j] = __funnelshift_rc(S[W0 + j], S[W0 + j + 1], dyn);
        if (32 * q < s.obs_stride) {
            int8_t *dg = obs_env + (size_t)ev.plist[li] * s.obs_stride + 32 * q;
            if (wide) st_global_256(dg, out);
            else {
                *reinterpret_cast<uint4 *>(dg) = make_uint4(out[0], out[1], out[2], out[3]);
                *reinterpret_cast<uint4 *>(dg + 16) = make_uint4(out[4], out[5], out[6], out[7]);
            }
        }
    }
}

template <int R>
__device__ void fast_obs_rows_lane(const DevSpec &s, const FastSpec &f, const Env &ev, const FastEnv &fe, int n_act, int8_t *obs_env,
                                   int tid, int T)
{
    constexpr int n = 2 * R + 1, NB = n * n;
    constexpr int RW = (n + 3) / 4;
    constexpr int LW = (n + 6) / 4;
    constexpr int NG = (NB + 63) / 64;
    const int pw4 = f.PW >> 2;
    const bool wide = ((s.obs_stride & 31) == 0) && ((reinterpret_cast<uintptr_t>(obs_env) & 31) == 0);
    for (int li = tid; li < n_act; li += T) {
        const int a = ev.ragent[li];
        const bool observing = ev.klass[a] & BGW_AG_OBSERVING;
        const int o = pad_index(s, f, ev.cell[a]) - R * f.PW - R;
        const uint32_t *wp = reinterpret_cast<const uint32_t *>(fe.cenc + (o & ~3));
        const int sh = (o & 3) * 8;
        int8_t *dst = obs_env + (size_t)ev.plist[li] * s.obs_stride;
#pragma unroll
        for (int g = 0; g < NG; ++g) {
            uint32_t out[16];
#pragma unroll
            for (int j = 0; j < 16; ++j) out[j] = 0;
            if (observing) {
#pragma unroll
                for (int i = 0; i < n; ++i) {
                    const int d = n * i;
                    if (d + n <= 64 * g || d >= 64 * (g + 1)) continue;
                    const uint32_t *rp = wp + i * pw4;
                    uint32_t x[LW + 1], y[RW];
#if defined(BGW_EXP_OBS1)
#pragma unroll
                    for (int j = 0; j < LW; ++j) x[j] = rp[0];
#else
#pragma unroll
                    for (int j = 0; j < LW; ++j) x[j] = (j < LW - 1 || sh + 8 * n > 32 * (LW - 1)) ? rp[j] : 0u;
#endif
                    x[LW] = 0;
#pragma unroll
                    for (int j = 0; j < RW; ++j) y[j] = __funnelshift_r(x[j], x[j + 1], sh);
                    constexpr int vb = n - 4 * (RW - 1);
                    if (vb < 4) y[RW - 1] &= (1u << (8 * (vb & 3))) - 1u;
                    const int q = (d >> 2) - 16 * g, s8 = (d & 3) * 8;
#pragma unroll
                    for (int j = 0; j < RW; ++j) {
                        if (q + j >= 0 && q + j < 16) out[q + j] |= y[j] << s8;
                        if (s8 != 0 && q + j + 1 >= 0 && q + j + 1 < 16) out[q + j + 1] |= y[j] >> (32 - s8);
                    }
                }
            }
            const int nchg = min(4, s.nchunks - 4 * g);
            int8_t *dg = dst + 64 * g;
#pragma unroll
            for (int h = 0; h < 2; ++h) {
                if (wide && nchg >= 2 * h + 2) st_global_256(dg + 32 * h, out + 8 * h);
                else {
                    if (nchg >= 2 * h + 1) *reinterpret_cast<uint4 *>(dg + 32 * h) = make_uint4(out[8 * h], out[8 * h + 1], out[8 * h + 2], out[8 * h + 3]);
                    if (nchg >= 2 * h + 2) *reinterpret_cast<uint4 *>(dg + 32 * h + 16) = make_uint4(out[8 * h + 4], out[8 * h + 5], out[8 * h + 6], out[8 * h + 7]);
                }
            }
        }
    }
}

template <int R>
__device__ __forceinline__ void fast_obs_rows(const DevSpec &s, const FastSpec &f, const Env &ev, const FastEnv &fe, int n_act, int8_t *obs_env,
                                              int tid, int T)
{
#ifndef BGW_OBS_ONE_LANE
    if constexpr (ObsCoop<R>::on) fast_obs_rows_coop<R>(s, f, ev, fe, n_act, obs_env, tid, T);
    else
#endif
        fast_obs_rows_lane<R>(s, f, ev, fe, n_act, obs_env, tid, T);
}

#ifndef BGW_C5_LB_N
#define BGW_C5_LB_N 8
#endif
#ifndef BGW_STATIC_T
#define BGW_STATIC_T 64
#endif
struct FastStaticC5 {
    static constexpr bool is_static = true;
    static constexpr int A = 256, L = 256, H = 64, W = 64, P = 5, PL = 5, PW = 76, PH = 74, obs_stride = 128, nchunks = 8,
                         obs_h = 11, view = 5, move_actor = BGW_MOVE_BOX, ravel = 0, observe_self = 1, done_mask = BGW_DONE_ONE_TEAM,
                         max_enc = 4, simd_ok = 1, async_ok = 1, slots = 256, T = BGW_STATIC_T, att = 1, identity = 1, can_mix = 0, acc_lt1 = 0, rpo = 0,
                         LB_T = BGW_STATIC_T, LB_N = BGW_C5_LB_N;
};
struct FastStaticC2 {
    static constexpr bool is_static = true;
    static constexpr int A = 24, L = 24, H = 8, W = 8, P = 3, PL = 3, PW = 16, PH = 14, obs_stride = 64, nchunks = 4,
                         obs_h = 7, view = 3, move_actor = BGW_MOVE_BOX, ravel = 0, observe_self = 1, done_mask = BGW_DONE_ONE_TEAM,
                         max_enc = 4, simd_ok = 1, async_ok = 2, slots = 64, T = 32, att = 1, identity = 1, can_mix = 0, acc_lt1 = 0, rpo = 0, LB_T = 128, LB_N = 7;
};
struct FastDynamic { static constexpr bool is_static = false; static constexpr int LB_T = 128, LB_N = 7; };

#ifndef __CUDACC_RTC__
template <typename C>
inline bool fast_shape_matches(const DevSpec &q, const FastSpec &f, int threads)
{
    return q.A == C::A && q.L == C::L && q.H == C::H && q.W == C::W && q.obs_stride == C::obs_stride && q.obs_h == C::obs_h &&
           q.obs_c == 1 && q.move_actor == C::move_actor && q.ravel == C::ravel && q.observe_self == C::observe_self &&
           q.done_mask == C::done_mask && q.max_enc == C::max_enc && f.P == C::P && f.PL == C::PL && f.PW == C::PW &&
           f.PH == C::PH && f.uniform_view == C::view && f.simd_ok == C::simd_ok && f.async_ok == C::async_ok &&
           q.slot_mask == C::slots - 1 && threads == C::T && f.uniform_att == C::att && f.identity_learners == C::identity &&
           f.can_mix == C::can_mix && f.acc_lt1 == C::acc_lt1 && q.randomize_placement_order == C::rpo;
}
#endif

#define BGW_FAST_LB __launch_bounds__(SHAPE::LB_T, SHAPE::LB_N)
template <typename SHAPE, typename HT>
__device__ __forceinline__ void bgw_step_fast_body(const DevSpec &s_in, const FastSpec &f_in, const BgwState &st, const uint32_t *actions,
                                                   uint32_t *sampled, const int16_t *order, int8_t *obs, float *reward, uint8_t *done,
                                                   uint8_t *all_done)
{
    DevSpec s = s_in;
    FastSpec f = f_in;
    if constexpr (SHAPE::is_static) {
        typedef SHAPE C;
        s.A = C::A; s.L = C::L; s.H = C::H; s.W = C::W; s.HW = C::H * C::W; s.obs_stride = C::obs_stride; s.nchunks = C::nchunks;
        s.obs_h = s.obs_w = C::obs_h; s.obs_c = 1; s.move_actor = C::move_actor; s.ravel = C::ravel; s.observe_self = C::observe_self;
        s.done_mask = C::done_mask; s.max_enc = C::max_enc; s.n_blk = 0; s.program = BGW_PROG_TEAM_BATTLE;
        s.randomize_placement_order = C::rpo;
        s.manager = BGW_MANAGER_ALL_STEP; s.attack_actor = BGW_ATTACK_BINARY; s.hw_words = (C::H * C::W + 31) / 32;
        f.P = C::P; f.PL = C::PL; f.PW = C::PW; f.PH = C::PH; f.uniform_view = C::view; f.simd_ok = C::simd_ok; f.async_ok = C::async_ok;
        f.uniform_att = C::att; f.identity_learners = C::identity; f.can_mix = C::can_mix; f.acc_lt1 = C::acc_lt1;
        f.magic_w = (uint32_t)(((1ull << 32) + C::W - 1) / C::W);
        s.slot_mask = C::slots - 1;
        constexpr FastLayout LY = fast_layout(C::A, C::L, C::H * C::W, C::PH, C::PW, C::slots, C::T, C::max_enc, (C::H * C::W + 31) / 32, C::identity);
        fast_apply_layout(f, LY);
    }
    int T_ = (int)blockDim.x;
    if constexpr (SHAPE::is_static) T_ = SHAPE::T;
    const int ptid = threadIdx.x, T = T_, lane = ptid & 31, nwarp = T >> 5;
    int tid = ptid, warp = ptid >> 5;
    unsigned char *scratch = bgw_smem + f.o_scratch;
    Env ev;
    ev.enc = (int8_t *)(bgw_smem + f.o_enc);
    ev.klass = bgw_smem + f.o_klass;
    ev.tmp = bgw_smem + f.o_tmp;
    ev.head = nullptr;
    ev.ragent = (uint16_t *)(bgw_smem + f.o_ragent);
    ev.plist = (uint16_t *)(bgw_smem + f.o_plist);
    ev.ctr = (int *)(bgw_smem + f.o_ctr);
    ev.racc = nullptr;
    ev.slot = (uint32_t *)(scratch + f.s_slot);
    ev.pstate = scratch + f.s_pstate;
    ev.avail = nullptr;
    ev.mask = nullptr; ev.act = nullptr;
    ev.ammo = nullptr;
    FastEnv fe;
    fe.head = bgw_smem + f.o_head;
    fe.rflag = scratch + f.s_rflag;
    fe.cenc = (int8_t *)(bgw_smem + f.o_cenc);
    fe.rel = (uint16_t *)(bgw_smem + f.o_rel);
    fe.act = (uint32_t *)(bgw_smem + f.o_act);
    fe.wsum = (int *)(bgw_smem + f.o_wsum);
    fe.rkmask = (uint32_t *)(scratch + f.s_rkmask);
    fe.eff = (uint16_t *)(scratch + f.s_eff);
    fe.killrank = (uint16_t *)(scratch + f.s_killrank);
    fe.touch = (uint32_t *)(scratch + f.s_touch);
    const double *rw = s.reward;
    const int nch = s.nchunks;

    if ((s.A & 3) == 0) {
        const uint32_t *e32 = (const uint32_t *)s.enc, *k32 = (const uint32_t *)s.klass;
        for (int w = tid; w < (s.A >> 2); w += T) {
            const uint32_t k = __ldg(&k32[w]);
            ((uint32_t *)ev.enc)[w] = __ldg(&e32[w]);
            ((uint32_t *)ev.klass)[w] = k;
        }
    } else {
        for (int a = tid; a < s.A; a += T) {
            const uint8_t k = __ldg(&s.klass[a]);
            ev.enc[a] = __ldg(&s.enc[a]); ev.klass[a] = k;
        }
    }
    uint32_t *const tk = f_in.ticket;
    const uint32_t NT = f_in.n_tickets, tbase = f_in.ticket_base;
    int *const tslot = fe.wsum + BGW_TSLOT;
    if (tid == 0) {
        const uint32_t g0 = tk ? atomicAdd(tk, 1u) - tbase : blockIdx.x;
        tslot[0] = (int)min(NT, g0);
        tslot[1] = (int)((g0 < NT) ? min(NT, tk ? atomicAdd(tk, 1u) - tbase : g0 + gridDim.x) : NT);
    }
    if (tid < 16) {
        double r = 0.0;
        if (tid & RF_ATTACK_FAIL) r += rw[BGW_RW_ATTACK_FAIL];
        if (tid & RF_KILL) r += rw[BGW_RW_KILL];
        if (tid & RF_DIED) r += rw[BGW_RW_DIE];
        if (tid & RF_MOVE_FAIL) r += rw[BGW_RW_MOVE_FAIL];
        r += rw[BGW_RW_ENTROPY];
        reinterpret_cast<float *>(fe.wsum + 16)[tid] = (float)r;
    }
    fast_init_dense(s, f, ev, fe, tid, T);
    asm volatile("griddepcontrol.launch_dependents;" ::: "memory");
    if (!f_in.chain) asm volatile("griddepcontrol.wait;" ::: "memory");

    uint32_t g = (uint32_t)tslot[0], gn = 0;
    int e = 0, kstep = 0, b = 0;
    uint8_t ef_cur = 0, ef_nxt = 0;
    uint32_t step_cur = 0, step_nxt = 0, epi_cur = 0, epi_nxt = 0;
    bool late = false;
    int kn_carry = 0, en_carry = 0;
    if (g < NT) {
        kstep = (int)(g / (uint32_t)s.E); e = (int)(g - (uint32_t)kstep * (uint32_t)s.E);
        kn_carry = kstep; en_carry = e;
        if (f_in.chain || kstep > 0) env_wait_stamp(f_in, e, f_in.seq + (uint32_t)kstep - 1u);
        fast_issue_env(s, f, st, actions, e, bgw_smem + f.o_buf, tid, T);
        ef_cur = __ldcg(&st.env_flags[e]); step_cur = __ldcg(&st.step[e]); epi_cur = __ldcg(&st.episode[e]);
    }
    cp_async_commit();

    uint32_t epoch = f_in.epoch0;
    int it_no = -1, sl = 1;
#ifndef BGW_STAMP_TID
#define BGW_STAMP_TID (T - 1)
#endif
    int pend_e = -1;
    uint32_t pend_v = 0;
#define BGW_FLUSH_STAMP()                                                            \
    do {                                                                             \
        if (pend_e >= 0) { st_release_u32(f_in.env_seq + pend_e, pend_v); pend_e = -1; } \
    } while (0)
#ifndef BGW_STAMP_DEFERRED
#define BGW_STAMP_ENV() st_release_u32(f_in.env_seq + e, f_in.seq + (uint32_t)kstep)
#else
#define BGW_STAMP_ENV() do { pend_e = e; pend_v = f_in.seq + (uint32_t)kstep; } while (0)
#endif
#define BGW_END_ENV()                                                                \
    do {                                                                             \
        if (tid == 0) tslot[sl ^ 1] = (int)tnew;                                     \
        __syncthreads();                                                             \
        BGW_JITTER_POINT(7);                                                         \
        if (tid == BGW_STAMP_TID) { BGW_FLUSH_STAMP(); BGW_STAMP_ENV(); }            \
        sl ^= 1;                                                                     \
    } while (0)
    for (; g < NT; g = gn) {
        ++it_no;
#ifdef BGW_WARP_ROTATION
        tid = ptid + 32 * (it_no % nwarp);
        if (tid >= T) tid -= T;
        warp = tid >> 5;
#endif
        BGW_PROF_MARK(0);
        kstep = kn_carry; e = en_carry;
        if (late) {
            BGW_FLUSH_STAMP();
            env_wait_stamp(f_in, e, f_in.seq + (uint32_t)kstep - 1u);
            fast_issue_env(s, f, st, actions, e, bgw_smem + f.o_buf + b * f.buf_bytes, tid, T);
            ef_cur = __ldcg(&st.env_flags[e]); step_cur = __ldcg(&st.step[e]); epi_cur = __ldcg(&st.episode[e]);
            cp_async_commit();
            late = false;
        }
        gn = (uint32_t)tslot[sl];
        uint32_t tnew = NT;
        BGW_JITTER_POINT(8);
        if (tid == 0 && gn < NT) tnew = min(NT, tk ? atomicAdd(tk, 1u) - tbase : gn + gridDim.x);
        if (gn < NT) {
            const int kn = (int)(gn / (uint32_t)s.E), en = (int)(gn - (uint32_t)kn * (uint32_t)s.E);
            kn_carry = kn; en_carry = en;
            if ((f_in.chain || kn > 0) && !env_stamped(f_in, en, f_in.seq + (uint32_t)kn - 1u)) late = true;
            else {
                fast_issue_env(s, f, st, actions, en, bgw_smem + f.o_buf + (b ^ 1) * f.buf_bytes, tid, T);
                ef_nxt = __ldcg(&st.env_flags[en]); step_nxt = __ldcg(&st.step[en]); epi_nxt = __ldcg(&st.episode[en]);
            }
        }
        cp_async_commit();

        unsigned char *buf = bgw_smem + f.o_buf + b * f.buf_bytes;
        ev.cell = (uint16_t *)(buf + f.b_cell);
        ev.next = (uint16_t *)(buf + f.b_next);
        ev.flags = buf + f.b_flags;
        ev.health = st.health + (size_t)e * s.A;
        for (int i = tid; i < (s.A * 8 + 127) / 128; i += T)
            asm volatile("prefetch.global.L2 [%0];" ::"l"((const char *)ev.health + (size_t)i * 128));
        ev.e = e; ev.genv = (uint32_t)(s.env_offset + e);
        int8_t *obs_env = obs ? obs + (size_t)e * s.L * s.obs_stride : nullptr;
        float *rew = reward + (size_t)e * s.L;
        uint8_t *dn = done + (size_t)e * s.L;
        const size_t off = (size_t)e * s.A;
        const uint8_t ef0 = ef_cur;
        ev.episode = epi_cur;
        ev.step = step_cur + 1u;
        b ^= 1; ef_cur = ef_nxt; step_cur = step_nxt; epi_cur = epi_nxt;

        if ((s.L & 15) == 0) {
            uint4 *d4 = (uint4 *)dn, *r4 = (uint4 *)rew;
            const uint4 z = make_uint4(0, 0, 0, 0);
            for (int i = tid; i < s.L / 16; i += T) d4[i] = z;
            for (int i = tid; i < s.L / 4; i += T) r4[i] = z;
        } else {
            for (int l = tid; l < s.L; l += T) { dn[l] = 0; rew[l] = 0.f; }
        }
        if (tid < CTR_COUNT) ev.ctr[tid] = 0;
        if (epoch < 4096u) {
            for (int i = tid; i <= s.slot_mask; i += T) ev.slot[i] = BGW_SLOT_FREE;
            epoch = 0xFFFFEu;
        }
        cp_async_wait<1>();
        __syncthreads();
        BGW_PROF_MARK(1);

        bool fresh = false;
        if (__builtin_expect((ef0 & BGW_ENV_ALL_DONE) != 0, 0)) {
            if (!s.auto_reset) {
                if (tid == 0) all_done[e] = ef0;
                BGW_END_ENV();
                continue;
            }
            {
                unsigned char *arena = bgw_smem + f.o_cenc;
                Env evr = ev;
                evr.head = (uint16_t *)arena;
                evr.racc = (double *)(arena + f.r_racc);
                evr.avail = (uint32_t *)(arena + f.r_avail);
                BgwState st_r = st;
                if constexpr (SHAPE::is_static) st_r.layout = nullptr;
                sim_reset(s, st_r, evr, tid, T);
                store_env(s, st, evr, true, tid, T);
                ev.episode = evr.episode; ev.step = evr.step;
            }
            const bool bad = ev.ctr[CTR_ERR] != 0;
            if (tid == 0) {
                const uint8_t fl = (uint8_t)((bad ? BGW_ENV_ERROR | BGW_ENV_ALL_DONE : 0) | BGW_ENV_RESET);
                st.error[e] = (uint32_t)ev.ctr[CTR_ERR];
                st.env_flags[e] = fl; all_done[e] = fl;
            }
            __syncthreads();
            fast_init_dense(s, f, ev, fe, tid, T);
            if (tid < CTR_COUNT) ev.ctr[tid] = 0;
            __syncthreads();
            if (bad) {
                if (obs_env)
                    for (int i = tid; i < s.L * nch; i += T) reinterpret_cast<uint4 *>(obs_env)[i] = make_uint4(0, 0, 0, 0);
                BGW_END_ENV();
                continue;
            }
            fresh = true;
        }
        BGW_PROF_MARK(2);

        int n_rel = 0, n_act = 0;
        if (f.simd_ok) {
            if (warp == BGW_COMPACT_WARP(T)) {
                const uint32_t *fw = (const uint32_t *)ev.flags, *kw = (const uint32_t *)ev.klass;
                const int nwords = s.A >> 2, wpl = (nwords + 31) >> 5;
                int cnt = 0;
                for (int j = 0; j < wpl; ++j) {
                    const int w = lane * wpl + j;
                    if (w < nwords) {
                        const uint32_t x = fw[w];
                        const uint32_t rel = ~__vcmpeq4(x & 0x07070707u, 0x04040404u);
                        const uint32_t act = __vcmpne4(kw[w] & (0x01010101u * BGW_AG_LEARNER), 0u) & __vcmpeq4(x & 0x04040404u, 0u);
                        cnt += (__popc(rel) >> 3) + ((__popc(act) >> 3) << 16);
                    }
                }
                int incl = cnt;
#pragma unroll
                for (int dd = 1; dd < 32; dd <<= 1) { const int t = __shfl_up_sync(0xFFFFFFFFu, incl, dd); if (lane >= dd) incl += t; }
                int pr = (incl - cnt) & 0xFFFF, pa = (incl - cnt) >> 16;
                const int tot = __shfl_sync(0xFFFFFFFFu, incl, 31);
                const bool same = f.identity_learners && (tot & 0xFFFF) == (tot >> 16);
                if (same) {
                    for (int j = 0; j < wpl; ++j) {
                        const int w = lane * wpl + j;
                        if (w < nwords) {
                            const uint32_t act = __vcmpeq4(fw[w] & 0x04040404u, 0u);
#pragma unroll
                            for (int bb = 0; bb < 4; ++bb)
                                if ((act >> (8 * bb)) & 1u) ev.ragent[pa++] = (uint16_t)(4 * w + bb);
                        }
                    }
                } else {
#pragma unroll 1
                    for (int j = 0; j < wpl; ++j) {
                        const int w = lane * wpl + j;
                        if (w < nwords) {
                            const uint32_t x = fw[w];
                            const uint32_t rel = ~__vcmpeq4(x & 0x07070707u, 0x04040404u);
                            const uint32_t act = __vcmpne4(kw[w] & (0x01010101u * BGW_AG_LEARNER), 0u) & __vcmpeq4(x & 0x04040404u, 0u);
#pragma unroll 1
                            for (int bb = 0; bb < 4; ++bb) {
                                const int a = 4 * w + bb;
                                if ((rel >> (8 * bb)) & 1u) fe.rel[pr++] = (uint16_t)a;
                                if ((act >> (8 * bb)) & 1u) ev.ragent[pa++] = (uint16_t)a;
                            }
                        }
                    }
                }
                if (lane == 31) fe.wsum[3] = same;
                if (lane == 31) { fe.wsum[0] = incl & 0xFFFF; fe.wsum[1] = incl >> 16; }
            }
            __syncthreads();
            n_rel = fe.wsum[0]; n_act = fe.wsum[1];
            fe.rel = fe.wsum[3] ? ev.ragent : (uint16_t *)(bgw_smem + f.o_rel);
        } else {
            for (int a0 = 0; a0 < s.A; a0 += T) {
                const int a = a0 + tid;
                bool rel = false, acting = false;
                if (a < s.A) {
                    const uint8_t fl = ev.flags[a];
                    rel = (fl & (BGW_ST_ACTIVE | BGW_ST_IN_GRID)) || !(fl & BGW_ST_DONE_REPORTED);
                    acting = (ev.klass[a] & BGW_AG_LEARNER) && !(fl & BGW_ST_DONE_REPORTED);
                }
                const unsigned br = __ballot_sync(0xFFFFFFFFu, rel), ba = __ballot_sync(0xFFFFFFFFu, acting);
                if (lane == 0) { fe.wsum[2 + warp] = __popc(br); fe.wsum[8 + warp] = __popc(ba); }
                __syncthreads();
                int before_r = n_rel, before_a = n_act;
                for (int w = 0; w < nwarp; ++w) {
                    const int cr = fe.wsum[2 + w], ca = fe.wsum[8 + w];
                    if (w < warp) { before_r += cr; before_a += ca; }
                    n_rel += cr; n_act += ca;
                }
                const unsigned lt = (1u << lane) - 1u;
                if (rel) fe.rel[before_r + __popc(br & lt)] = (uint16_t)a;
                if (acting) ev.ragent[before_a + __popc(ba & lt)] = (uint16_t)a;
                __syncthreads();
            }
        }
        if (order) {
            n_act = 0;
            for (int i0 = 0; i0 < s.L; i0 += T) {
                const int i = i0 + tid;
                int a = 0;
                bool acting = false;
                if (i < s.L) {
                    a = __ldg(&s.agent_of[order[(size_t)e * s.L + i]]);
                    acting = !(ev.flags[a] & BGW_ST_DONE_REPORTED);
                }
                __syncthreads();
                const unsigned ba = __ballot_sync(0xFFFFFFFFu, acting);
                if (lane == 0) fe.wsum[2 + warp] = __popc(ba);
                __syncthreads();
                int before = n_act;
                for (int w = 0; w < nwarp; ++w) { const int c = fe.wsum[2 + w]; if (w < warp) before += c; n_act += c; }
                if (acting) ev.ragent[before + __popc(ba & ((1u << lane) - 1u))] = (uint16_t)a;
            }
            __syncthreads();
        }
        BGW_PROF_MARK(3);

        for (int x = tid; x < n_rel; x += T) {
            const int a = fe.rel[x];
            fe.rflag[a] = 0;
            fe.killrank[a] = BGW_NONE16;
            if (ev.flags[a] & BGW_ST_IN_GRID) {
                if (ev.next[a] != BGW_NONE16) ev.tmp[ev.next[a]] = 1;
                fe.cenc[pad_index(s, f, ev.cell[a])] = ev.enc[a];
            }
        }
        __syncthreads();
        for (int x = tid; x < n_rel; x += T) {
            const int a = fe.rel[x];
            if (ev.flags[a] & BGW_ST_IN_GRID) {
                if (!ev.tmp[a]) ((HT *)fe.head)[ev.cell[a]] = (HT)a;
                ev.tmp[a] = 0;
                const int p = pad_index(s, f, ev.cell[a]);
                if (f.can_mix && fe.cenc[p] != ev.enc[a]) { fe.cenc[p] = (int8_t)BGW_MIXED; ev.ctr[CTR_MIXED] = 1; }
            }
        }
        __syncthreads();
        BGW_PROF_MARK(4);

        if (fresh) {
            for (int i = tid; i < n_act; i += T) ev.plist[i] = f.identity_learners ? ev.ragent[i] : (uint16_t)__ldg(&s.learner_of[ev.ragent[i]]);
            if (!f.identity_learners) __syncthreads();
        } else {
            for (int i = tid; i < n_act; i += T) {
                const int a = ev.ragent[i], l = f.identity_learners ? a : __ldg(&s.learner_of[a]);
                ev.plist[i] = (uint16_t)l;
                if (sampled) {
                    const uint32_t w = sample_action_word(s, a, ev.klass[a], ev.genv, ev.episode, ev.step - 1u);
                    fe.act[l] = w;
                    sampled[(size_t)e * s.L + l] = w;
                } else {
                    fe.act[l] = __ldcg(&actions[(size_t)e * s.L + l]);
                }
                uint8_t p = 0;
                if ((ev.flags[a] & BGW_ST_ACTIVE) && (ev.klass[a] & BGW_AG_ATTACKING) && (int8_t)((fe.act[l] >> 16) & 0xFF) != 0) {
                    const int R = f.uniform_att >= 0 ? f.uniform_att : __ldg(&s.attack_r[a]), n = 2 * R + 1;
                    const unsigned long long row = __ldg(&s.attack_map[ev.enc[a]]);
                    const int wo = pad_index(s, f, ev.cell[a]) - R * f.PW - R;
                    const int8_t *w = fe.cenc + wo;
                    uint32_t mask = 0;
                    if (R == 1) {
                        const uint32_t *wp = reinterpret_cast<const uint32_t *>(fe.cenc + (wo & ~3));
                        const int sh = (wo & 3) * 8, pw4 = f.PW >> 2;
                        uint32_t y[3];
    #pragma unroll
                        for (int k = 0; k < 3; ++k) y[k] = __funnelshift_r(wp[k * pw4], wp[k * pw4 + 1], sh);
                        if (s.max_enc < 32) {
                            const uint32_t row32 = (uint32_t)row & ~1u;
    #pragma unroll
                            for (int k = 0; k < 9; ++k) {
                                const uint32_t v = (y[k / 3] >> (8 * (k % 3))) & 0xFFu;
                                mask |= (__funnelshift_rc(row32, 0u, v) & 1u) << k;
                            }
                        } else {
    #pragma unroll
                            for (int k = 0; k < 9; ++k) {
                                const uint32_t v = (y[k / 3] >> (8 * (k % 3))) & 0xFFu;
                                if (v < 64u && ((row >> v) & 1ull)) mask |= 1u << k;
                            }
                        }
                        if (f.can_mix && ev.ctr[CTR_MIXED]) {
    #pragma unroll
                            for (int k = 0; k < 9; ++k)
                                if (((y[k / 3] >> (8 * (k % 3))) & 0xFFu) == (uint32_t)(uint8_t)BGW_MIXED) mask |= 1u << k;
                        }
                    } else {
                        for (int wr = 0; wr < n; ++wr)
                            for (int wc = 0; wc < n; ++wc) {
                                const int v = w[wr * f.PW + wc];
                                if (v > 0 ? (int)((row >> v) & 1ull) : (v == BGW_MIXED)) mask |= 1u << (wr * n + wc);
                            }
                    }
                    fe.rkmask[i] = mask;
                    if (mask) {
                        p = 1; fe.eff[atomicAdd(&ev.ctr[CTR_NEMIT], 1)] = (uint16_t)i;
                        const SlotTables stt = slot_tables(s, ev);
                        attack_reserve(s, stt.t0, stt.mask, ev.cell[a], R, mask, (epoch << BGW_TAG_SHIFT) | (uint32_t)i);
                    }
                    else p = 3;
                }
                ev.pstate[i] = p;
            }
            __syncthreads();
            BGW_PROF_MARK(5);
            {
                const int n_eff = ev.ctr[CTR_NEMIT];
                if (n_eff > 0) {
                    if (warp == BGW_ROUNDS_WARP(T)) {
                        const uint32_t e2 = fast_attack_rounds<true, HT>(s, f, ev, fe, n_eff, epoch, lane, T);
                        if (lane == 0) ev.ctr[CTR_EPOCH] = (int)e2;
                    }
                    __syncthreads();
                    epoch = (uint32_t)ev.ctr[CTR_EPOCH];
                }
                else --epoch;
            }
            BGW_PROF_MARK(6);

            int pend = 0;
            for (int i = tid; i < n_act; i += T) {
                const int a = ev.ragent[i];
                const bool active = ev.flags[a] & BGW_ST_ACTIVE;
                if (ev.pstate[i] == 3) {
                    const unsigned kr = fe.killrank[a];
                    if (active || (kr != BGW_NONE16 && kr > (unsigned)i)) fe.rflag[a] |= RF_ATTACK_FAIL;
                }
                uint32_t ft = BGW_NO_MOVE;
                if (active) {
                    bool ok = false;
                    if (ev.klass[a] & BGW_AG_MOVING) {
                        int dr, dc, r0, c0;
                        const int from = ev.cell[a];
                        decode_move(s, a, fe.act[ev.plist[i]], dr, dc);
                        cell_rc(s, f, from, r0, c0);
                        const int r = r0 + dr, c = c0 + dc;
                        if (r >= 0 && r < s.H && c >= 0 && c < s.W) {
                            if (dr == 0 && dc == 0) ok = true;
                            else ft = ((uint32_t)from << 16) | (uint32_t)(r * s.W + c);
                        }
                    }
                    if (ft == BGW_NO_MOVE && !ok) fe.rflag[a] |= RF_MOVE_FAIL;
                }
                fe.rkmask[i] = ft;
                if (ft != BGW_NO_MOVE) {
                    touch_mark(f, fe, (int)(ft >> 16));
                    touch_mark(f, fe, (int)(ft & 0xFFFFu));
                    pend = 1;
                }
            }
            pend = __syncthreads_or(pend);
            BGW_PROF_MARK(7);
            if (pend) epoch = fast_move_phase<HT>(s, f, ev, fe, n_act, epoch, tid, T);
            BGW_PROF_MARK(8);

            BGW_FLUSH_STAMP();
            for (int i = tid; i < n_act; i += T) {
                const int a = ev.ragent[i], l = ev.plist[i];
                const unsigned rf = fe.rflag[a];
                const bool dd = prog_done(s, ev, a);
                rew[l] = reinterpret_cast<const float *>(fe.wsum + 16)[rf & 15u];
                dn[l] = (uint8_t)(BGW_OUT_VALID | (dd ? BGW_OUT_DONE : 0));
                if (dd) ev.flags[a] |= BGW_ST_DONE_REPORTED; else atomicAdd(&ev.ctr[CTR_REMAINING], 1);
            }
        }
        if (!fresh)
            for (int x = tid; x < n_rel; x += T) {
                const int a = fe.rel[x];
                if (racc_persists(ev.klass[a]) && (fe.rflag[a] & RF_DIED)) st.reward_acc[off + a] = __ldcg(&st.reward_acc[off + a]) + rw[BGW_RW_DIE];
            }
        BGW_PROF_MARK(9);

        if (obs_env) {
            const bool direct = s.observe_self && !(f.can_mix && ev.ctr[CTR_MIXED]);
            const int R = direct ? f.uniform_view : -1;
            switch (R) {
            case 1: fast_obs_rows<1>(s, f, ev, fe, n_act, obs_env, tid, T); break;
            case 2: fast_obs_rows<2>(s, f, ev, fe, n_act, obs_env, tid, T); break;
            case 3: fast_obs_rows<3>(s, f, ev, fe, n_act, obs_env, tid, T); break;
            case 4: fast_obs_rows<4>(s, f, ev, fe, n_act, obs_env, tid, T); break;
            case 5: fast_obs_rows<5>(s, f, ev, fe, n_act, obs_env, tid, T); break;
            default: {
                const int items = n_act * nch;
                for (int it = tid; it < items; it += T) {
                    const int li = it / nch, ch = it - li * nch;
                    const int l = ev.plist[li], a = ev.ragent[li];
                    uint32_t w[4];
                    fast_obs_chunk_slow<HT>(s, f, ev, fe, a, ch, w);
                    *reinterpret_cast<uint4 *>(obs_env + (size_t)l * s.obs_stride + ch * 16) = make_uint4(w[0], w[1], w[2], w[3]);
                }
            }
            }
        }
        __syncthreads();
        BGW_PROF_MARK(10);

        {
            uint32_t lo = 0, hi = 0;
            int ok = 1;
            for (int x = tid; x < n_rel; x += T) {
                const int a = fe.rel[x];
                const uint8_t fl = ev.flags[a];
                if (!fresh) { st.cell[off + a] = ev.cell[a]; st.next[off + a] = ev.next[a]; st.flags[off + a] = fl; }
                if (fl & BGW_ST_ACTIVE) { const int en2 = ev.enc[a]; if (en2 < 32) lo |= 1u << en2; else hi |= 1u << (en2 - 32); }
                if (s.done_mask & (BGW_DONE_TARGET_AGENT | BGW_DONE_TARGET_DESTROYED)) {
                    const int t = __ldg(&s.target[a]);
                    if ((s.done_mask & BGW_DONE_TARGET_AGENT) && t >= 0 && !same_position(ev, a, t)) ok = 0;
                    if ((s.done_mask & BGW_DONE_TARGET_DESTROYED) && t >= 0 && (ev.flags[t] & BGW_ST_ACTIVE)) ok = 0;
                }
                if (fl & BGW_ST_IN_GRID) fe.cenc[pad_index(s, f, ev.cell[a])] = 0;
            }
            lo = __reduce_or_sync(0xFFFFFFFFu, lo);
            hi = __reduce_or_sync(0xFFFFFFFFu, hi);
            ok = __all_sync(0xFFFFFFFFu, ok);
            if (lane == 0) {
                if (lo) atomicOr((unsigned *)&ev.ctr[CTR_ENC_LO], lo);
                if (hi) atomicOr((unsigned *)&ev.ctr[CTR_ENC_HI], hi);
                if (!ok) atomicOr((unsigned *)&ev.ctr[CTR_AND], 1u);
            }
        }
        __syncthreads();
        if (tid == BGW_BOOK_TID && !fresh) {
            const unsigned long long encs = ((unsigned long long)(unsigned)ev.ctr[CTR_ENC_HI] << 32) | (unsigned)ev.ctr[CTR_ENC_LO];
            int d = !ev.ctr[CTR_AND];
            if (s.done_mask & BGW_DONE_ACTIVE) d &= (encs == 0);
            if (s.done_mask & BGW_DONE_ONE_TEAM) d &= ((encs & (encs - 1)) == 0);
            uint8_t ef = 0;
            if (d || ev.ctr[CTR_REMAINING] == 0) ef |= BGW_ENV_ALL_DONE;
            if (s.horizon > 0 && (int)ev.step >= s.horizon) ef |= BGW_ENV_ALL_DONE | BGW_ENV_TRUNCATED;
            st.step[e] = ev.step;
            st.env_flags[e] = ef;
            all_done[e] = ef;
            unsigned long long *sr = (unsigned long long *)st.stats + (size_t)e * BGW_STAT_COUNT;
            atomicAdd(&sr[BGW_STAT_AGENT_STEPS], (unsigned long long)n_act);
            atomicAdd(&sr[BGW_STAT_ENV_STEPS], 1ull);
            if (ev.ctr[CTR_KILLS]) atomicAdd(&sr[BGW_STAT_KILLS], (unsigned long long)ev.ctr[CTR_KILLS]);
            if (ef & BGW_ENV_ALL_DONE) atomicAdd(&sr[BGW_STAT_EPISODES], 1ull);
        }
        BGW_END_ENV();
        BGW_PROF_MARK(11);
    }
    BGW_FLUSH_STAMP();
#undef BGW_END_ENV
#undef BGW_STAMP_ENV
#undef BGW_FLUSH_STAMP
    cp_async_wait<0>();
}

template <typename SHAPE, typename HT>
__global__ void BGW_FAST_LB bgw_step_fast_kernel(const DevSpec s_in, const FastSpec f_in, const BgwState st, const uint32_t *actions,
                                     uint32_t *sampled, const int16_t *order, int8_t *obs, float *reward, uint8_t *done,
                                     uint8_t *all_done)
{
    bgw_step_fast_body<SHAPE, HT>(s_in, f_in, st, actions, sampled, order, obs, reward, done, all_done);
}

#ifdef BGW_SMALL_KERNELS
struct ObserveLayout { int o_cell, o_flags, o_klass, o_enc, o_ragent, o_plist, bytes; };
inline __host__ __device__ ObserveLayout observe_layout(int A, int L, int PH, int PW)
{
    ObserveLayout o;
    int off = (PH * PW + 32 + 15) & ~15;
    o.o_cell = off;   off += ((A + 7) & ~7) * 2;
    o.o_ragent = off; off += ((L + 7) & ~7) * 2;
    o.o_plist = off;  off += ((L + 7) & ~7) * 2;
    o.o_flags = off;  off += (A + 15) & ~15;
    o.o_klass = off;  off += (A + 15) & ~15;
    o.o_enc = off;    off += (A + 15) & ~15;
    o.bytes = off;
    return o;
}

template <int R>
__global__ void __launch_bounds__(128) bgw_observe_fast_kernel(const DevSpec s, const FastSpec f, const BgwState st, const uint8_t *env_mask,
                                                               int8_t *obs)
{
    const int tid = threadIdx.x, T = blockDim.x;
    const ObserveLayout lay = observe_layout(s.A, s.L, f.PH, f.PW);
    Env ev;
    FastEnv fe;
    fe.cenc = (int8_t *)bgw_smem;
    ev.cell = (uint16_t *)(bgw_smem + lay.o_cell);
    ev.ragent = (uint16_t *)(bgw_smem + lay.o_ragent);
    ev.plist = (uint16_t *)(bgw_smem + lay.o_plist);
    ev.flags = bgw_smem + lay.o_flags;
    ev.klass = bgw_smem + lay.o_klass;
    ev.enc = (int8_t *)(bgw_smem + lay.o_enc);
    {
        uint32_t *c32 = (uint32_t *)fe.cenc;
        const int wpr = f.PW >> 2;
        const int rows_per_pass = wpr <= T ? T / wpr : 1;
        const int r0 = wpr <= T ? tid / wpr : 0;
        for (int cw = wpr <= T ? tid - r0 * wpr : tid; cw < wpr && r0 < rows_per_pass; cw += T) {
            uint32_t inner = 0xFFFFFFFFu;
            for (int bb = 0; bb < 4; ++bb) {
                const int cc = cw * 4 + bb;
                if (cc >= f.PL && cc < f.PL + s.W) inner &= ~(0xFFu << (8 * bb));
            }
            for (int rr = r0; rr < f.PH; rr += rows_per_pass) c32[rr * wpr + cw] = (rr >= f.P && rr < f.P + s.H) ? inner : 0xFFFFFFFFu;
        }
        if (tid < 8) c32[f.PH * wpr + tid] = 0xFFFFFFFFu;
        for (int a = tid; a < s.A; a += T) { ev.klass[a] = __ldg(&s.klass[a]); ev.enc[a] = __ldg(&s.enc[a]); }
        for (int l = tid; l < s.L; l += T) { ev.ragent[l] = (uint16_t)__ldg(&s.agent_of[l]); ev.plist[l] = (uint16_t)l; }
    }
    __syncthreads();
    for (int e = blockIdx.x; e < s.E; e += gridDim.x) {
        if (env_mask && !env_mask[e]) continue;
        const size_t off = (size_t)e * s.A;
        for (int a = tid; a < s.A; a += T) {
            const uint16_t c = __ldcs(&st.cell[off + a]);
            const uint8_t fl = __ldcs(&st.flags[off + a]);
            ev.cell[a] = c; ev.flags[a] = fl;
            if (fl & BGW_ST_IN_GRID) fe.cenc[pad_index(s, f, c)] = ev.enc[a];
        }
        __syncthreads();
        fast_obs_rows<R>(s, f, ev, fe, s.L, obs + (size_t)e * s.L * s.obs_stride, tid, T);
        __syncthreads();
        for (int a = tid; a < s.A; a += T)
            if (ev.flags[a] & BGW_ST_IN_GRID) fe.cenc[pad_index(s, f, ev.cell[a])] = 0;
        __syncthreads();
    }
}
#endif
```

### abmarl_b200/csrc/bgw_fastk.cu

```cuda
#include "bgw_dev.cuh"
#include "bgw_fast.cuh"

const void *bgw_fast_step_fn(int shape, int head_elem)
{
    if (shape == 1) return (const void *)bgw_step_fast_kernel<FastStaticC5, uint8_t>;
    if (shape == 2) return (const void *)bgw_step_fast_kernel<FastStaticC2, uint8_t>;
    if (head_elem == 1) return (const void *)bgw_step_fast_kernel<FastDynamic, uint8_t>;
    return (const void *)bgw_step_fast_kernel<FastDynamic, uint16_t>;
}
```

Before: 13.25 billion.

## Shrink fast-kernel shared memory with narrower rank/mask types and reused tmp buffer

Drops the dedicated tmp buffer (aliased into scratch pstate and the rel area), stores actions as 16-bit, and for compile-time shapes uses 8-bit ranks and 16-bit move/attack masks. Move entries now store only the destination and recompute the source cell from the agent. The aim is a smaller per-CTA shared-memory footprint so more CTAs fit per SM, with a static_assert guarding 12 CTAs/SM for the C5 shape. It adds a relayout on every specialize/fallback path and relies on narrower types staying within range, including the killrank sentinel now that its reset is removed.

```diff
diff --git a/abmarl_b200/csrc/bgw.cu b/abmarl_b200/csrc/bgw.cu
--- a/abmarl_b200/csrc/bgw.cu
+++ b/abmarl_b200/csrc/bgw.cu
@@ -90,6 +90,14 @@
 };
 
 namespace {
+
+void fast_relayout(BgwEngine *h, bool compile_time_shape)
+{
+    const DevSpec &q = h->dsf;
+    FastSpec &f = h->fs;
+    fast_apply_layout(f, fast_layout(q.A, q.L, q.HW, f.PH, f.PW, q.slot_mask + 1, q.max_enc, q.hw_words, f.identity_learners,
+                                     compile_time_shape && fast_rank8(q.L), compile_time_shape && fast_mask16(f.uniform_att)));
+}
 
 template <typename T>
 int upload(BgwEngine *h, const T *src, size_t n, const T **dst)
@@ -417,9 +425,7 @@
             h->dsf = d;
             h->dsf.slot_mask = fslots - 1;
             const long long cbytes = (long long)f.PH * f.PW + 32;
-            const FastLayout ly = fast_layout(A, L, HW, f.PH, f.PW, fslots, TF, max_enc, d.hw_words, L == A);
-            fast_apply_layout(f, ly);
-            const int fo = ly.smem_bytes;
+            const int fo = fast_layout(A, L, HW, f.PH, f.PW, fslots, max_enc, d.hw_words, L == A, false, false).smem_bytes;
             f.async_ok = (A % 16 == 0) ? 1 : (A % 8 == 0) ? 2 : 0;
             f.simd_ok = (A % 4 == 0);
             f.uniform_view = -1;
@@ -459,6 +465,7 @@
         if (fast) {
             h->fast_shape = fast_shape_matches<FastStaticC5>(h->dsf, f, TF) ? 1 : fast_shape_matches<FastStaticC2>(h->dsf, f, TF) ? 2 : 0;
             if (const char *t = getenv("BGW_DYNAMIC_SHAPES")) if (atoi(t)) h->fast_shape = 0;
+            fast_relayout(h, h->fast_shape != 0);
             h->fast_fn = bgw_fast_step_fn(h->fast_shape, f.head_elem);
         }
     }
@@ -558,18 +565,24 @@
             return fail(2, "bgw_specialize: %s", e);
         return 0;
     }
+    int per_sm = 0, sms = 0;
+    CUDA_OK(cudaDeviceGetAttribute(&sms, cudaDevAttrMultiProcessorCount, h->device));
+    fast_relayout(h, true);
     const int by_smem = (228 * 1024) / (h->fs.smem_bytes + 1024), by_regs = 65536 / (h->threads_fast * 72);
     const int lb_n = std::max(1, std::min(32, std::min(by_smem, by_regs)));
-    if (const char *e = bgwjit::build_fast(h->dsf, h->fs, h->threads_fast, lb_n, cache_dir, h->fast_jit, msg))
+    if (const char *e = bgwjit::build_fast(h->dsf, h->fs, h->threads_fast, lb_n, cache_dir, h->fast_jit, msg)) {
+        fast_relayout(h, false);
         return fail(2, "bgw_specialize: %s", e);
-    int per_sm = 0, sms = 0;
+    }
     const int rc = bgwjit::driver().OccupancyMaxActiveBlocks(&per_sm, h->fast_jit.function, h->threads_fast, (size_t)h->fs.smem_bytes);
-    if (rc || per_sm < 1) { bgwjit::driver().ModuleUnload(h->fast_jit.module); h->fast_jit = bgwjit::Kernel(); return fail(2, "bgw_specialize: occupancy query of the compiled kernel failed (%d)", rc); }
-    CUDA_OK(cudaDeviceGetAttribute(&sms, cudaDevAttrMultiProcessorCount, h->device));
+    if (rc || per_sm < 1) {
+        bgwjit::driver().ModuleUnload(h->fast_jit.module); h->fast_jit = bgwjit::Kernel(); fast_relayout(h, false);
+        return fail(2, "bgw_specialize: occupancy query of the compiled kernel failed (%d)", rc);
+    }
     h->fs.grid_ctas = std::max(1, std::min(h->ds.E, per_sm * sms));
     if (const char *t = getenv("BGW_GRID")) { const int v = atoi(t); if (v >= 1) h->fs.grid_ctas = std::min(h->ds.E, v); }
     h->fast_jit_on = true;
-    if (getenv("BGW_VERBOSE")) fprintf(stderr, "[bgw] fast kernel compiled for this spec's shape: %d CTAs/SM, grid=%d\n", per_sm, h->fs.grid_ctas);
+    if (getenv("BGW_VERBOSE")) fprintf(stderr, "[bgw] fast kernel compiled for this spec's shape: smem=%d B/CTA, %d CTAs/SM, grid=%d\n", h->fs.smem_bytes, per_sm, h->fs.grid_ctas);
     return 0;
 }
 
@@ -607,6 +620,7 @@
         h->fast_jit_on = false;
         DeviceGuard guard(h->device);
         h->fast_shape = 0;
+        fast_relayout(h, false);
         h->fast_fn = bgw_fast_step_fn(0, h->fs.head_elem);
         CUDA_OK(cudaFuncSetAttribute(h->fast_fn, cudaFuncAttributeMaxDynamicSharedMemorySize, h->fs.smem_bytes));
         int per_sm = 0, sms = 0;
diff --git a/abmarl_b200/csrc/bgw_fast.cuh b/abmarl_b200/csrc/bgw_fast.cuh
--- a/abmarl_b200/csrc/bgw_fast.cuh
+++ b/abmarl_b200/csrc/bgw_fast.cuh
@@ -33,7 +33,7 @@
     int simd_ok;
     uint32_t epoch0;
     int b_cell, b_next, b_flags, buf_bytes;
-    int o_enc, o_klass, o_tmp, o_act, o_head, o_cenc, o_rel, o_ragent, o_plist, o_ctr, o_wsum, o_buf, o_scratch;
+    int o_enc, o_klass, o_act, o_head, o_cenc, o_rel, o_ragent, o_plist, o_ctr, o_wsum, o_buf, o_scratch;
     int s_rflag, s_slot, s_rkmask, s_eff, s_pstate, s_killrank, s_touch, scratch_bytes, smem_bytes;
     int touch_words;
     int r_racc, r_avail;
@@ -50,7 +50,7 @@
 
 struct FastLayout {
     int b_cell, b_next, b_flags, buf_bytes;
-    int o_enc, o_klass, o_tmp, o_act, o_head, o_cenc, o_rel, o_ragent, o_plist, o_ctr, o_wsum, o_buf, o_scratch;
+    int o_enc, o_klass, o_act, o_head, o_cenc, o_rel, o_ragent, o_plist, o_ctr, o_wsum, o_buf, o_scratch;
     int s_rflag, s_slot, s_rkmask, s_eff, s_pstate, s_killrank, s_touch, touch_words, scratch_bytes, smem_bytes;
     int r_racc, r_avail, head_elem;
 };
@@ -63,19 +63,21 @@
     return w;
 }
 
-__host__ __device__ constexpr FastLayout fast_layout(int A, int L, int HW, int PH, int PW, int slots, int T, int max_enc,
-                                                     int hw_words, int identity)
+__host__ __device__ constexpr bool fast_rank8(int L) { return L <= 256; }
+__host__ __device__ constexpr bool fast_mask16(int att) { return att >= 0 && att <= 1; }
+
+__host__ __device__ constexpr FastLayout fast_layout(int A, int L, int HW, int PH, int PW, int slots, int max_enc, int hw_words,
+                                                     int identity, bool rank8, bool mask16)
 {
     FastLayout y{};
     int fo = 0;
     y.o_enc = fo; fo += fl_align16(A);
     y.o_klass = fo; fo += fl_align16(A);
-    y.o_tmp = fo; fo += fl_align16(A);
     y.o_rel = fo; fo += fl_align16(A * 2);
     y.o_ragent = fo; fo += fl_align16(L * 2);
     y.o_plist = identity ? y.o_ragent : fo;
     if (!identity) fo += fl_align16(L * 2);
-    y.o_act = fo; fo += fl_align16(L * 4);
+    y.o_act = fo; fo += fl_align16(L * 2);
     y.o_ctr = fo; fo += fl_align16(CTR_COUNT * 4);
     y.o_wsum = fo; fo += fl_align16(32 * 4);
     int bo = 0;
@@ -85,10 +87,10 @@
     y.buf_bytes = bo;
     y.o_buf = fo; fo += 2 * bo;
     int so = 0;
-    y.s_rkmask = so; so += fl_align16(L * 4);
-    y.s_eff = so; so += fl_align16(L * 2);
-    y.s_pstate = so; so += fl_align16(L);
-    y.s_killrank = so; so += fl_align16(A * 2);
+    y.s_rkmask = so; so += fl_align16(L * (mask16 ? 2 : 4));
+    y.s_eff = so; so += fl_align16(L * (rank8 ? 1 : 2));
+    y.s_pstate = so; so += fl_align16(A);
+    y.s_killrank = so; so += fl_align16(A * (rank8 ? 1 : 2));
     y.s_slot = so; so += fl_align16(slots * 4);
     y.touch_words = fl_touch_words(HW);
     y.s_touch = so; so += 2 * y.touch_words * 4;
@@ -113,7 +115,7 @@
 __host__ __device__ inline void fast_apply_layout(FastSpec &f, const FastLayout &y)
 {
     f.b_cell = y.b_cell; f.b_next = y.b_next; f.b_flags = y.b_flags; f.buf_bytes = y.buf_bytes;
-    f.o_enc = y.o_enc; f.o_klass = y.o_klass; f.o_tmp = y.o_tmp; f.o_act = y.o_act; f.o_head = y.o_head;
+    f.o_enc = y.o_enc; f.o_klass = y.o_klass; f.o_act = y.o_act; f.o_head = y.o_head;
     f.o_cenc = y.o_cenc; f.o_rel = y.o_rel; f.o_ragent = y.o_ragent; f.o_plist = y.o_plist; f.o_ctr = y.o_ctr;
     f.o_wsum = y.o_wsum; f.o_buf = y.o_buf; f.o_scratch = y.o_scratch;
     f.s_rflag = y.s_rflag; f.s_slot = y.s_slot; f.s_rkmask = y.s_rkmask; f.s_eff = y.s_eff; f.s_pstate = y.s_pstate;
@@ -127,11 +129,40 @@
     void *head;
     uint8_t *rflag;
     int8_t *cenc;
-    uint16_t *killrank, *eff, *rel;
-    uint32_t *rkmask, *act;
+    uint16_t *rel;
+    uint16_t *act;
     uint32_t *touch;
     int *wsum;
 };
+
+template <typename RT, typename MT>
+struct FastRanks {
+    typedef RT rank_t;
+    typedef MT mask_t;
+    RT *eff;
+    RT *killrank;
+    MT *rkmask;
+    static constexpr MT no_move = (MT)~0u;
+};
+
+template <bool B, typename X, typename Y> struct fl_pick { typedef X type; };
+template <typename X, typename Y> struct fl_pick<false, X, Y> { typedef Y type; };
+template <typename SHAPE, bool = SHAPE::is_static>
+struct FastWidths {
+    static constexpr bool rank8 = false, mask16 = false;
+    typedef FastRanks<uint16_t, uint32_t> Ranks;
+};
+template <typename SHAPE>
+struct FastWidths<SHAPE, true> {
+    static constexpr bool rank8 = fast_rank8(SHAPE::L), mask16 = fast_mask16(SHAPE::att);
+    typedef FastRanks<typename fl_pick<rank8, uint8_t, uint16_t>::type, typename fl_pick<mask16, uint16_t, uint32_t>::type> Ranks;
+};
+template <typename C>
+__host__ __device__ constexpr FastLayout fast_static_layout()
+{
+    return fast_layout(C::A, C::L, C::H * C::W, C::PH, C::PW, C::slots, C::max_enc, (C::H * C::W + 31) / 32, C::identity,
+                       FastWidths<C>::rank8, FastWidths<C>::mask16);
+}
 
 __device__ __forceinline__ void cell_rc(const DevSpec &s, const FastSpec &f, int cell, int &r, int &c)
 {
@@ -273,8 +304,8 @@
     }
 }
 
-template <typename HT>
-__device__ void fast_exec_attack(const DevSpec &s, const FastSpec &f, Env &ev, FastEnv &fe, int rank, int a, uint32_t mask)
+template <typename HT, typename FR>
+__device__ void fast_exec_attack(const DevSpec &s, const FastSpec &f, Env &ev, FastEnv &fe, const FR &rk, int rank, int a, uint32_t mask)
 {
     if (!(ev.flags[a] & BGW_ST_ACTIVE)) return;
     const int R = f.uniform_att >= 0 ? f.uniform_att : __ldg(&s.attack_r[a]), n = 2 * R + 1;
@@ -305,7 +336,7 @@
     }
     if (!(ev.flags[v] & BGW_ST_ACTIVE)) {
         fe.cenc[pad_index(s, f, vcell)] = fl_summary(ev, fl_unlink<HT>(ev, fe, v), f.can_mix);
-        fe.killrank[v] = (uint16_t)rank;
+        rk.killrank[v] = (typename FR::rank_t)rank;
         atomicAdd(&ev.ctr[CTR_KILLS], 1);
         fe.rflag[v] |= RF_DIED;
         fe.rflag[a] |= RF_KILL;
@@ -365,8 +396,9 @@
 #define BGW_COMPACT_WARP(T) 0
 #endif
 
-template <bool WARP, typename HT>
-__device__ uint32_t fast_attack_rounds(const DevSpec &s, const FastSpec &f, Env &ev, FastEnv &fe, int n_eff, uint32_t epoch, int tid, int T)
+template <bool WARP, typename HT, typename FR>
+__device__ uint32_t fast_attack_rounds(const DevSpec &s, const FastSpec &f, Env &ev, FastEnv &fe, const FR &rk, int n_eff, uint32_t epoch,
+                                       int tid, int T)
 {
     const int stride = WARP ? 32 : T;
     const SlotTables st = slot_tables(s, ev);
@@ -375,17 +407,17 @@
         const uint32_t tag = epoch << BGW_TAG_SHIFT, next_tag = (epoch - 1u) << BGW_TAG_SHIFT;
         int lost = 0;
         for (int x = tid; x < n_eff; x += stride) {
-            const int i = fe.eff[x];
+            const int i = rk.eff[x];
             if (ev.pstate[i] != 1) continue;
             const int a = ev.ragent[i], R = f.uniform_att >= 0 ? f.uniform_att : __ldg(&s.attack_r[a]), own = ev.cell[a];
-            const uint32_t mask = fe.rkmask[i];
+            const uint32_t mask = rk.rkmask[i];
             if (!attack_holds(s, st.tab(p), st.mask, own, R, mask, tag | (uint32_t)i)) {
                 lost = 1;
                 attack_reserve(s, st.tab(p ^ 1), st.mask, own, R, mask, next_tag | (uint32_t)i);
                 continue;
             }
             BGW_JITTER_POINT(9);
-            fast_exec_attack<HT>(s, f, ev, fe, i, a, mask);
+            fast_exec_attack<HT>(s, f, ev, fe, rk, i, a, mask);
             ev.pstate[i] = 0;
         }
         if (WARP) { pending = __any_sync(0xFFFFFFFFu, lost); __syncwarp(); } else pending = __syncthreads_or(lost);
@@ -423,7 +455,6 @@
     if (f.can_mix && ns == (int8_t)BGW_MIXED) ev.ctr[CTR_MIXED] = 1;
 }
 
-#define BGW_NO_MOVE 0xFFFFFFFFu
 __device__ __forceinline__ void touch_mark(const FastSpec &f, FastEnv &fe, int cell)
 {
     BGW_JITTER_POINT(3);
@@ -432,8 +463,9 @@
     if (atomicOr(w, bit) & bit) atomicOr(w + f.touch_words, bit);
 }
 
-template <bool WARP, typename HT>
-__device__ uint32_t fast_move_rounds(const DevSpec &s, const FastSpec &f, Env &ev, FastEnv &fe, int n_cur, uint32_t epoch, int tid, int T)
+template <bool WARP, typename HT, typename FR>
+__device__ uint32_t fast_move_rounds(const DevSpec &s, const FastSpec &f, Env &ev, FastEnv &fe, const FR &rk, int n_cur, uint32_t epoch,
+                                     int tid, int T)
 {
     const int stride = WARP ? 32 : T;
     const SlotTables st = slot_tables(s, ev);
@@ -442,15 +474,14 @@
     int pending = 1;
     while (pending) {
         const uint32_t tag = epoch << BGW_TAG_SHIFT, next_tag = (epoch - 1u) << BGW_TAG_SHIFT;
-        const uint16_t *walk = which ? fe.killrank : fe.eff;
-        uint16_t *losers = which ? fe.eff : fe.killrank;
+        const typename FR::rank_t *walk = which ? rk.killrank : rk.eff;
+        typename FR::rank_t *losers = which ? rk.eff : rk.killrank;
         int *lctr = &ev.ctr[CTR_PA + (which ^ 1)];
         const int lbase = which ? base0 : base1;
         int lost = 0;
         for (int x = tid; x < n_cur; x += stride) {
             const int i = walk[x];
-            const uint32_t ft = fe.rkmask[i];
-            const int from = (int)(ft >> 16), to = (int)(ft & 0xFFFFu);
+            const int a = ev.ragent[i], from = ev.cell[a], to = rk.rkmask[i];
             const uint32_t mine = tag | (uint32_t)i, sf = (uint32_t)from & st.mask, sto = (uint32_t)to & st.mask;
             BGW_JITTER_POINT(4);
             const uint32_t hf = cur[sf], ht = cur[sto];
@@ -458,10 +489,10 @@
                 lost = 1;
                 atomicMin(&nxt[sf], next_tag | (uint32_t)i);
                 atomicMin(&nxt[sto], next_tag | (uint32_t)i);
-                losers[atomicAdd(lctr, 1) - lbase] = (uint16_t)i;
+                losers[atomicAdd(lctr, 1) - lbase] = (typename FR::rank_t)i;
                 continue;
             }
-            fast_exec_move<HT>(s, f, ev, fe, ev.ragent[i], from, to);
+            fast_exec_move<HT>(s, f, ev, fe, a, from, to);
         }
         if (WARP) { pending = __any_sync(0xFFFFFFFFu, lost); __syncwarp(); }
         else pending = __syncthreads_or(lost);
@@ -474,24 +505,25 @@
     return epoch;
 }
 
-template <typename HT>
-__device__ uint32_t fast_move_phase(const DevSpec &s, const FastSpec &f, Env &ev, FastEnv &fe, int n_act, uint32_t epoch, int tid, int T)
+template <typename HT, typename FR>
+__device__ uint32_t fast_move_phase(const DevSpec &s, const FastSpec &f, Env &ev, FastEnv &fe, const FR &rk, int n_act, uint32_t epoch,
+                                    int tid, int T)
 {
     const SlotTables st = slot_tables(s, ev);
     const uint32_t *twice = fe.touch + f.touch_words;
     const uint32_t tw = (uint32_t)f.touch_words - 1u, tag = epoch << BGW_TAG_SHIFT;
     for (int i = tid; i < n_act; i += T) {
-        const uint32_t ft = fe.rkmask[i];
-        if (ft == BGW_NO_MOVE) continue;
-        const int from = (int)(ft >> 16), to = (int)(ft & 0xFFFFu);
+        const typename FR::mask_t dst = rk.rkmask[i];
+        if (dst == FR::no_move) continue;
+        const int a = ev.ragent[i], from = ev.cell[a], to = dst;
         BGW_JITTER_POINT(5);
         const uint32_t c = (twice[((uint32_t)from >> 5) & tw] >> (from & 31)) | (twice[((uint32_t)to >> 5) & tw] >> (to & 31));
         if (c & 1u) {
-            fe.eff[atomicAdd(&ev.ctr[CTR_PA], 1)] = (uint16_t)i;
+            rk.eff[atomicAdd(&ev.ctr[CTR_PA], 1)] = (typename FR::rank_t)i;
             atomicMin(&st.t0[(uint32_t)from & st.mask], tag | (uint32_t)i);
             atomicMin(&st.t0[(uint32_t)to & st.mask], tag | (uint32_t)i);
         } else {
-            fast_exec_move<HT>(s, f, ev, fe, ev.ragent[i], from, to);
+            fast_exec_move<HT>(s, f, ev, fe, a, from, to);
         }
     }
     __syncthreads();
@@ -502,7 +534,7 @@
     const int n_con = ev.ctr[CTR_PA];
     if (n_con > 0) {
         if ((tid >> 5) == BGW_ROUNDS_WARP(T)) {
-            const uint32_t e2 = fast_move_rounds<true, HT>(s, f, ev, fe, n_con, epoch, tid & 31, T);
+            const uint32_t e2 = fast_move_rounds<true, HT>(s, f, ev, fe, rk, n_con, epoch, tid & 31, T);
             if ((tid & 31) == 0) ev.ctr[CTR_EPOCH] = (int)e2;
         }
         __syncthreads();
@@ -811,9 +843,10 @@
         f.uniform_att = C::att; f.identity_learners = C::identity; f.can_mix = C::can_mix; f.acc_lt1 = C::acc_lt1;
         f.magic_w = (uint32_t)(((1ull << 32) + C::W - 1) / C::W);
         s.slot_mask = C::slots - 1;
-        constexpr FastLayout LY = fast_layout(C::A, C::L, C::H * C::W, C::PH, C::PW, C::slots, C::T, C::max_enc, (C::H * C::W + 31) / 32, C::identity);
+        constexpr FastLayout LY = fast_static_layout<C>();
         fast_apply_layout(f, LY);
     }
+    typedef typename FastWidths<SHAPE>::Ranks FR;
     int T_ = (int)blockDim.x;
     if constexpr (SHAPE::is_static) T_ = SHAPE::T;
     const int ptid = threadIdx.x, T = T_, lane = ptid & 31, nwarp = T >> 5;
@@ -822,7 +855,7 @@
     Env ev;
     ev.enc = (int8_t *)(bgw_smem + f.o_enc);
     ev.klass = bgw_smem + f.o_klass;
-    ev.tmp = bgw_smem + f.o_tmp;
+    ev.tmp = scratch + f.s_pstate;
     ev.head = nullptr;
     ev.ragent = (uint16_t *)(bgw_smem + f.o_ragent);
     ev.plist = (uint16_t *)(bgw_smem + f.o_plist);
@@ -838,12 +871,13 @@
     fe.rflag = scratch + f.s_rflag;
     fe.cenc = (int8_t *)(bgw_smem + f.o_cenc);
     fe.rel = (uint16_t *)(bgw_smem + f.o_rel);
-    fe.act = (uint32_t *)(bgw_smem + f.o_act);
+    fe.act = (uint16_t *)(bgw_smem + f.o_act);
     fe.wsum = (int *)(bgw_smem + f.o_wsum);
-    fe.rkmask = (uint32_t *)(scratch + f.s_rkmask);
-    fe.eff = (uint16_t *)(scratch + f.s_eff);
-    fe.killrank = (uint16_t *)(scratch + f.s_killrank);
     fe.touch = (uint32_t *)(scratch + f.s_touch);
+    FR rk;
+    rk.eff = (typename FR::rank_t *)(scratch + f.s_eff);
+    rk.killrank = (typename FR::rank_t *)(scratch + f.s_killrank);
+    rk.rkmask = (typename FR::mask_t *)(scratch + f.s_rkmask);
     const double *rw = s.reward;
     const int nch = s.nchunks;
 
@@ -978,6 +1012,7 @@
             for (int l = tid; l < s.L; l += T) { dn[l] = 0; rew[l] = 0.f; }
         }
         if (tid < CTR_COUNT) ev.ctr[tid] = 0;
+        for (int w = tid; w < (s.A + 3) >> 2; w += T) reinterpret_cast<uint32_t *>(ev.tmp)[w] = 0u;
         if (epoch < 4096u) {
             for (int i = tid; i <= s.slot_mask; i += T) ev.slot[i] = BGW_SLOT_FREE;
             epoch = 0xFFFFEu;
@@ -996,6 +1031,7 @@
             {
                 unsigned char *arena = bgw_smem + f.o_cenc;
                 Env evr = ev;
+                evr.tmp = bgw_smem + f.o_rel;
                 evr.head = (uint16_t *)arena;
                 evr.racc = (double *)(arena + f.r_racc);
                 evr.avail = (uint32_t *)(arena + f.r_avail);
@@ -1128,7 +1164,6 @@
         for (int x = tid; x < n_rel; x += T) {
             const int a = fe.rel[x];
             fe.rflag[a] = 0;
-            fe.killrank[a] = BGW_NONE16;
             if (ev.flags[a] & BGW_ST_IN_GRID) {
                 if (ev.next[a] != BGW_NONE16) ev.tmp[ev.next[a]] = 1;
                 fe.cenc[pad_index(s, f, ev.cell[a])] = ev.enc[a];
@@ -1139,7 +1174,6 @@
             const int a = fe.rel[x];
             if (ev.flags[a] & BGW_ST_IN_GRID) {
                 if (!ev.tmp[a]) ((HT *)fe.head)[ev.cell[a]] = (HT)a;
-                ev.tmp[a] = 0;
                 const int p = pad_index(s, f, ev.cell[a]);
                 if (f.can_mix && fe.cenc[p] != ev.enc[a]) { fe.cenc[p] = (int8_t)BGW_MIXED; ev.ctr[CTR_MIXED] = 1; }
             }
@@ -1154,15 +1188,16 @@
             for (int i = tid; i < n_act; i += T) {
                 const int a = ev.ragent[i], l = f.identity_learners ? a : __ldg(&s.learner_of[a]);
                 ev.plist[i] = (uint16_t)l;
+                uint32_t aw;
                 if (sampled) {
-                    const uint32_t w = sample_action_word(s, a, ev.klass[a], ev.genv, ev.episode, ev.step - 1u);
-                    fe.act[l] = w;
-                    sampled[(size_t)e * s.L + l] = w;
+                    aw = sample_action_word(s, a, ev.klass[a], ev.genv, ev.episode, ev.step - 1u);
+                    sampled[(size_t)e * s.L + l] = aw;
                 } else {
-                    fe.act[l] = __ldcg(&actions[(size_t)e * s.L + l]);
-                }
+                    aw = __ldcg(&actions[(size_t)e * s.L + l]);
+                }
+                fe.act[l] = (uint16_t)aw;
                 uint8_t p = 0;
-                if ((ev.flags[a] & BGW_ST_ACTIVE) && (ev.klass[a] & BGW_AG_ATTACKING) && (int8_t)((fe.act[l] >> 16) & 0xFF) != 0) {
+                if ((ev.flags[a] & BGW_ST_ACTIVE) && (ev.klass[a] & BGW_AG_ATTACKING) && (int8_t)((aw >> 16) & 0xFF) != 0) {
                     const int R = f.uniform_att >= 0 ? f.uniform_att : __ldg(&s.attack_r[a]), n = 2 * R + 1;
                     const unsigned long long row = __ldg(&s.attack_map[ev.enc[a]]);
                     const int wo = pad_index(s, f, ev.cell[a]) - R * f.PW - R;
@@ -1200,9 +1235,9 @@
                                 if (v > 0 ? (int)((row >> v) & 1ull) : (v == BGW_MIXED)) mask |= 1u << (wr * n + wc);
                             }
                     }
-                    fe.rkmask[i] = mask;
+                    rk.rkmask[i] = (typename FR::mask_t)mask;
                     if (mask) {
-                        p = 1; fe.eff[atomicAdd(&ev.ctr[CTR_NEMIT], 1)] = (uint16_t)i;
+                        p = 1; rk.eff[atomicAdd(&ev.ctr[CTR_NEMIT], 1)] = (typename FR::rank_t)i;
                         const SlotTables stt = slot_tables(s, ev);
                         attack_reserve(s, stt.t0, stt.mask, ev.cell[a], R, mask, (epoch << BGW_TAG_SHIFT) | (uint32_t)i);
                     }
@@ -1216,7 +1251,7 @@
                 const int n_eff = ev.ctr[CTR_NEMIT];
                 if (n_eff > 0) {
                     if (warp == BGW_ROUNDS_WARP(T)) {
-                        const uint32_t e2 = fast_attack_rounds<true, HT>(s, f, ev, fe, n_eff, epoch, lane, T);
+                        const uint32_t e2 = fast_attack_rounds<true, HT>(s, f, ev, fe, rk, n_eff, epoch, lane, T);
                         if (lane == 0) ev.ctr[CTR_EPOCH] = (int)e2;
                     }
                     __syncthreads();
@@ -1230,36 +1265,33 @@
             for (int i = tid; i < n_act; i += T) {
                 const int a = ev.ragent[i];
                 const bool active = ev.flags[a] & BGW_ST_ACTIVE;
-                if (ev.pstate[i] == 3) {
-                    const unsigned kr = fe.killrank[a];
-                    if (active || (kr != BGW_NONE16 && kr > (unsigned)i)) fe.rflag[a] |= RF_ATTACK_FAIL;
-                }
-                uint32_t ft = BGW_NO_MOVE;
+                if (ev.pstate[i] == 3 && (active || rk.killrank[a] > (unsigned)i)) fe.rflag[a] |= RF_ATTACK_FAIL;
+                const int from = ev.cell[a];
+                int to = -1;
                 if (active) {
                     bool ok = false;
                     if (ev.klass[a] & BGW_AG_MOVING) {
                         int dr, dc, r0, c0;
-                        const int from = ev.cell[a];
                         decode_move(s, a, fe.act[ev.plist[i]], dr, dc);
                         cell_rc(s, f, from, r0, c0);
                         const int r = r0 + dr, c = c0 + dc;
                         if (r >= 0 && r < s.H && c >= 0 && c < s.W) {
                             if (dr == 0 && dc == 0) ok = true;
-                            else ft = ((uint32_t)from << 16) | (uint32_t)(r * s.W + c);
+                            else to = r * s.W + c;
                         }
                     }
-                    if (ft == BGW_NO_MOVE && !ok) fe.rflag[a] |= RF_MOVE_FAIL;
-                }
-                fe.rkmask[i] = ft;
-                if (ft != BGW_NO_MOVE) {
-                    touch_mark(f, fe, (int)(ft >> 16));
-                    touch_mark(f, fe, (int)(ft & 0xFFFFu));
+                    if (to < 0 && !ok) fe.rflag[a] |= RF_MOVE_FAIL;
+                }
+                rk.rkmask[i] = to < 0 ? FR::no_move : (typename FR::mask_t)to;
+                if (to >= 0) {
+                    touch_mark(f, fe, from);
+                    touch_mark(f, fe, to);
                     pend = 1;
                 }
             }
             pend = __syncthreads_or(pend);
             BGW_PROF_MARK(7);
-            if (pend) epoch = fast_move_phase<HT>(s, f, ev, fe, n_act, epoch, tid, T);
+            if (pend) epoch = fast_move_phase<HT>(s, f, ev, fe, rk, n_act, epoch, tid, T);
             BGW_PROF_MARK(8);
 
             BGW_FLUSH_STAMP();
diff --git a/abmarl_b200/csrc/bgw_fastk.cu b/abmarl_b200/csrc/bgw_fastk.cu
--- a/abmarl_b200/csrc/bgw_fastk.cu
+++ b/abmarl_b200/csrc/bgw_fastk.cu
@@ -1,5 +1,7 @@
 #include "bgw_dev.cuh"
 #include "bgw_fast.cuh"
+
+static_assert(fast_static_layout<FastStaticC5>().smem_bytes <= 233472 / 12 - 1024, "FastStaticC5 no longer fits 12 CTAs per SM");
 
 const void *bgw_fast_step_fn(int shape, int head_elem)
 {
```

Result: faster. 13.55 billion (median of 6 runs) (+2.3%).
